# vincentherrmann/constrastive-predictive-coding-audio

Measured on NVIDIA B200. Metric: train audio-sec/sec, higher is better.
Workload: dtype f32

## Files before the change

### constrastive-predictive-coding-audio_b200/cpc_b200/ops.py

```python
import contextlib
import ctypes

import torch
from torch.autograd.function import once_differentiable

from . import _lib

_PRECISION = {"fp32": 0, "bf16": 1}
_default_precision = "fp32"


def set_default_precision(name):
    global _default_precision
    if name not in _PRECISION:
        raise ValueError(name)
    _default_precision = name


def get_default_precision():
    return _default_precision


def strict_fp32_libraries():
    torch.backends.cudnn.allow_tf32 = False
    torch.backends.cuda.matmul.allow_tf32 = False


_second_order = False


@contextlib.contextmanager
def second_order(enabled=True):
    global _second_order
    previous, _second_order = _second_order, bool(enabled)
    try:
        yield
    finally:
        _second_order = previous


def second_order_enabled():
    return _second_order


kernel_switches = {}
_CONV_SWITCHES = (("CPC_FORCE_CUDA_CORE_CONV", _lib.CONV_FLAG_CUDA_CORE), ("CPC_NO_TALL_CONV", _lib.CONV_FLAG_NO_TALL),
                  ("CPC_NO_SMALLK_CONV", _lib.CONV_FLAG_NO_SMALLK), ("CPC_NO_FUSED_DGRAD", _lib.CONV_FLAG_NO_FUSED_DGRAD),
                  ("CPC_NO_MMA_SMALL_WGRAD", _lib.CONV_FLAG_NO_MMA_SMALL_WGRAD))


def _switch(name):
    import os
    if name in kernel_switches:
        return bool(kernel_switches[name])
    return os.environ.get(name) == "1"


switch = _switch


def _conv_flags():
    flags = 0
    for name, bit in _CONV_SWITCHES:
        if _switch(name):
            flags |= bit
    return flags


def _require_cuda(*tensors):
    for t in tensors:
        if t is not None and not t.is_cuda:
            raise _lib.CpcError("cpc_b200 ops need CUDA tensors on a B200 (sm_100a); got a %s tensor and there is "
                                "no CPU fallback" % t.device.type)


def _ptr(t):
    return ctypes.c_void_p(t.data_ptr()) if t is not None else ctypes.c_void_p(0)


def _stream():
    return ctypes.c_void_p(torch.cuda.current_stream().cuda_stream)


class KernelProfiler:

    def __init__(self):
        self.records = []

    def __enter__(self):
        global _profiler
        _profiler = self
        return self

    def __exit__(self, *exc):
        global _profiler
        _profiler = None

    def summary(self):
        torch.cuda.synchronize()
        agg = {}
        for key, flops, nbytes, e0, e1 in self.records:
            a = agg.setdefault(key, {"key": key, "count": 0, "total_ms": 0.0, "flops_per_launch": flops,
                                     "bytes_per_launch": nbytes})
            a["count"] += 1
            a["total_ms"] += e0.elapsed_time(e1)
        total = sum(a["total_ms"] for a in agg.values()) or 1.0
        out = sorted(agg.values(), key=lambda a: -a["total_ms"])
        for a in out:
            a["avg_ms"] = a["total_ms"] / a["count"]
            a["share"] = a["total_ms"] / total
            a["tflops"] = a["flops_per_launch"] / (a["avg_ms"] * 1e-3) / 1e12 if a["avg_ms"] > 0 else 0.0
            a["gbs"] = a["bytes_per_launch"] / (a["avg_ms"] * 1e-3) / 1e9 if a["avg_ms"] > 0 else 0.0
        return out


_profiler = None


def _call(key, flops, fn, *args, nbytes=0.0):
    if _profiler is None:
        status = fn(*args)
    else:
        e0, e1 = torch.cuda.Event(enable_timing=True), torch.cuda.Event(enable_timing=True)
        e0.record()
        status = fn(*args)
        e1.record()
        _profiler.records.append((key, flops, nbytes, e0, e1))
    _lib.check(status, key.split(" ")[0])


CONV_FAMILIES = {0: "conv_tiled_cuda_core", 1: "conv_small_k_direct", 2: "tall_conv_tcgen05_32ch", 3: "tall_conv_tcgen05_128ch",
                 4: "conv_implicit_gemm_tcgen05"}


def _conv_key(tag, p):
    which = {"cpc_conv_fwd": 0, "cpc_conv_dgrad": 1, "cpc_conv_wgrad": 2}[tag]
    fam = CONV_FAMILIES.get(_lib.load().cpc_conv_kernel_family(ctypes.byref(p), which), "?")
    return "%s b%d %dx%dx%d->%dx%dx%d k%dx%d s%dx%d [%s]" % (tag, p.batch, p.c_in, p.h_in, p.w_in, p.c_out, p.h_out,
                                                            p.w_out, p.kh, p.kw, p.stride_h, p.stride_w, fam)


def _conv_flops(p):
    return 2.0 * p.c_out * p.c_in * p.kh * p.kw * p.batch * p.h_out * p.w_out


def _workspace(nbytes, device):
    if nbytes == 0:
        return None
    return torch.empty(int(nbytes), dtype=torch.uint8, device=device)



_OVERLAP_MAX_FLOPS = 60e9
_side_streams = {}


def _side_stream(device):
    key = (device.type, device.index)
    if key not in _side_streams:
        _side_streams[key] = torch.cuda.Stream(device=device)
    return _side_streams[key]


def _conv_params(x_shape, w_shape, stride, pad_top, pad_left, out_hw, relu, precision):
    p = _lib.ConvParams()
    p.batch, p.c_in, p.h_in, p.w_in = x_shape
    p.c_out, _, p.kh, p.kw = w_shape
    p.h_out, p.w_out = out_hw
    p.stride_h, p.stride_w = stride
    p.pad_top, p.pad_left = pad_top, pad_left
    p.relu = int(relu)
    p.precision = _PRECISION[precision]
    p.flags = _conv_flags()
    return p


def _pack_operand(lib, t, p, operand):
    nbytes = lib.cpc_conv_packed_bytes(ctypes.byref(p), operand)
    if nbytes == 0:
        return None
    packed = torch.empty(int(nbytes), dtype=torch.uint8, device=t.device)
    _call("cpc_conv_pack %s" % ("x" if operand == 0 else "dy"), 0.0, lib.cpc_conv_pack, _ptr(t), _ptr(packed), ctypes.byref(p),
          operand, _stream(), nbytes=4.0 * t.numel() + float(nbytes))
    return packed


class _ConvFunction(torch.autograd.Function):
    @staticmethod
    def forward(ctx, x, weight, bias, stride, pad_top, pad_left, out_hw, relu, precision):
        y, saved = _conv_forward(ctx, x, weight, bias, stride, pad_top, pad_left, out_hw, relu, precision)
        ctx.save_for_backward(*saved)
        return y

    @staticmethod
    def backward(ctx, dy):
        return _conv_backward(ctx, ctx.saved_tensors, dy) + (None,) * 6


class _ConvPoolFunction(torch.autograd.Function):

    @staticmethod
    def forward(ctx, x, weight, bias, stride, pad_top, pad_left, out_hw, relu, precision, kernel, ceil_mode):
        y, saved = _conv_forward(ctx, x, weight, bias, stride, pad_top, pad_left, out_hw, relu, precision)
        lib = _lib.load()
        x = saved[0]
        p = _pool_params(tuple(x.shape), kernel, ceil_mode)
        if p.h_out <= 0 or p.w_out <= 0:
            raise ValueError("max_pool2d output would be empty for input %s, kernel %d" % (tuple(x.shape), kernel))
        pooled = torch.empty((p.batch, p.channels, p.h_out, p.w_out), dtype=torch.float32, device=x.device)
        with torch.cuda.device(x.device):
            _call("cpc_maxpool_fwd b%d %dx%dx%d k%d" % (p.batch, p.channels, p.h_in, p.w_in, kernel), 0.0,
                  lib.cpc_maxpool_fwd, _ptr(x), _ptr(pooled), ctypes.byref(p), _stream(),
                  nbytes=4.0 * (x.numel() + pooled.numel()))
        ctx.pool = (kernel, ceil_mode)
        ctx.set_materialize_grads(False)
        ctx.save_for_backward(*saved)
        return y, pooled

    @staticmethod
    @once_differentiable
    def backward(ctx, dy, d_pooled):
        saved = ctx.saved_tensors
        x = saved[0]
        kernel, ceil_mode = ctx.pool
        lib = _lib.load()
        dx = dw = db = None
        if dy is not None:
            dx, dw, db = _conv_backward(ctx, saved, dy)
        if d_pooled is not None and ctx.needs_input_grad[0]:
            p = _pool_params(tuple(x.shape), kernel, ceil_mode)
            d_pooled = d_pooled.contiguous()
            with torch.cuda.device(x.device):
                if dx is None:
                    dx = torch.empty_like(x)
                    _call("cpc_maxpool_bwd b%d %dx%dx%d k%d" % (p.batch, p.channels, p.h_in, p.w_in, kernel), 0.0,
                          lib.cpc_maxpool_bwd, _ptr(x), _ptr(d_pooled), _ptr(dx), ctypes.byref(p), _stream(),
                          nbytes=4.0 * (2 * x.numel() + d_pooled.numel()))
                else:
                    _call("cpc_maxpool_bwd b%d %dx%dx%d k%d +=" % (p.batch, p.channels, p.h_in, p.w_in, kernel), 0.0,
                          lib.cpc_maxpool_bwd_accumulate, _ptr(x), _ptr(d_pooled), _ptr(dx), ctypes.byref(p), _stream(),
                          nbytes=4.0 * (3 * x.numel() + d_pooled.numel()))
        return (dx, dw, db) + (None,) * 8


def _conv_forward(ctx, x, weight, bias, stride, pad_top, pad_left, out_hw, relu, precision):
    _require_cuda(x, weight, bias)
    lib = _lib.load()
    x = x.contiguous()
    w = weight.contiguous()
    if x.dtype != torch.float32 or w.dtype != torch.float32:
        raise _lib.CpcError("conv expects fp32 tensors (precision is a kernel-internal setting)")
    p = _conv_params(tuple(x.shape), tuple(w.shape), stride, pad_top, pad_left, out_hw, relu, precision)
    y = torch.empty((x.shape[0], w.shape[0], out_hw[0], out_hw[1]), dtype=torch.float32, device=x.device)
    ws = _workspace(lib.cpc_conv_workspace_bytes(ctypes.byref(p), 0), x.device)
    with torch.cuda.device(x.device):
        keep = ctx.needs_input_grad[1]
        packed_x = _pack_operand(lib, x, p, 0) if keep else None
        _call(_conv_key("cpc_conv_fwd", p), _conv_flops(p), lib.cpc_conv_fwd_ex, _ptr(x), _ptr(w),
              _ptr(bias.contiguous() if bias is not None else None), _ptr(y), ctypes.byref(p), _ptr(packed_x),
              _ptr(ws), ws.numel() if ws is not None else 0, _stream())
    ctx.params = (tuple(x.shape), tuple(w.shape), stride, pad_top, pad_left, out_hw, precision)
    ctx.has_bias = bias is not None
    ctx.relu = relu
    return y, (x, w, y if relu else None, packed_x)


def _conv_backward(ctx, saved, dy):
    x, w, y, packed_x = saved
    lib = _lib.load()
    x_shape, w_shape, stride, pad_top, pad_left, out_hw, precision = ctx.params
    if ctx.relu:
        dy = dy * (y > 0).to(dy.dtype) if torch.is_grad_enabled() else torch.ops.aten.threshold_backward(dy, y, 0.0)
    dy = dy.contiguous()
    if torch.is_grad_enabled():
        geom = (x_shape, w_shape, stride, pad_top, pad_left, out_hw, precision)
        dx = _ConvDgradFunction.apply(dy, w, geom) if ctx.needs_input_grad[0] else None
        dw = _ConvWgradFunction.apply(x, dy, geom) if ctx.needs_input_grad[1] else None
        db = dy.sum(dim=(0, 2, 3)) if (ctx.has_bias and ctx.needs_input_grad[2]) else None
        return dx, dw, db
    p = _conv_params(x_shape, w_shape, stride, pad_top, pad_left, out_hw, False, precision)
    dx = dw = db = None
    need_dx = ctx.needs_input_grad[0]
    need_dw = ctx.needs_input_grad[1] or (ctx.has_bias and ctx.needs_input_grad[2])
    with torch.cuda.device(dy.device):
        packed_dy = None
        if need_dw:
            nbytes = lib.cpc_conv_packed_bytes(ctypes.byref(p), 1)
            if nbytes and ctx.has_bias:
                packed_dy = torch.empty(int(nbytes), dtype=torch.uint8, device=dy.device)
                db = torch.empty(w_shape[0], dtype=torch.float32, device=dy.device)
                _call("cpc_conv_pack dy", 0.0, lib.cpc_conv_pack_dy, _ptr(dy), _ptr(packed_dy), _ptr(db), ctypes.byref(p),
                      _stream(), nbytes=4.0 * dy.numel() + float(nbytes))
            else:
                packed_dy = _pack_operand(lib, dy, p, 1)
        side = None
        if need_dx and need_dw and _profiler is None and _conv_flops(p) < _OVERLAP_MAX_FLOPS and not _switch("CPC_NO_BWD_OVERLAP"):
            side = _side_stream(dy.device)
            side.wait_stream(torch.cuda.current_stream(dy.device))
        ws_d = ws_w = None
        if need_dx:
            dx = torch.empty(x_shape, dtype=torch.float32, device=dy.device)
            ws_d = _workspace(lib.cpc_conv_workspace_bytes(ctypes.byref(p), 1), dy.device)
            _call(_conv_key("cpc_conv_dgrad", p), _conv_flops(p), lib.cpc_conv_dgrad_ex, _ptr(dy), _ptr(w), _ptr(dx),
                  ctypes.byref(p), _ptr(packed_dy), _ptr(ws_d), ws_d.numel() if ws_d is not None else 0, _stream())
        if need_dw:
            dw = torch.empty(w_shape, dtype=torch.float32, device=dy.device)
            db_here = None
            if ctx.has_bias and db is None:
                db = db_here = torch.empty(w_shape[0], dtype=torch.float32, device=dy.device)
            ws_w = _workspace(lib.cpc_conv_workspace_bytes(ctypes.byref(p), 2), dy.device)
            with (torch.cuda.stream(side) if side is not None else contextlib.nullcontext()):
                _call(_conv_key("cpc_conv_wgrad", p), _conv_flops(p), lib.cpc_conv_wgrad_ex, _ptr(x), _ptr(dy), _ptr(dw),
                      _ptr(db_here), ctypes.byref(p), _ptr(packed_x), _ptr(packed_dy), _ptr(ws_w),
                      ws_w.numel() if ws_w is not None else 0, _stream())
        if side is not None:
            torch.cuda.current_stream(dy.device).wait_stream(side)
    return dx, dw, db


class _ConvDgradFunction(torch.autograd.Function):

    @staticmethod
    def forward(ctx, dy, w, geom):
        _require_cuda(dy, w)
        lib = _lib.load()
        x_shape, w_shape, stride, pad_top, pad_left, out_hw, precision = geom
        dy, w = dy.contiguous(), w.contiguous()
        p = _conv_params(x_shape, w_shape, stride, pad_top, pad_left, out_hw, False, precision)
        dx = torch.empty(x_shape, dtype=torch.float32, device=dy.device)
        ws = _workspace(lib.cpc_conv_workspace_bytes(ctypes.byref(p), 1), dy.device)
        with torch.cuda.device(dy.device):
            _call(_conv_key("cpc_conv_dgrad", p), _conv_flops(p), lib.cpc_conv_dgrad_ex, _ptr(dy), _ptr(w), _ptr(dx),
                  ctypes.byref(p), _ptr(None), _ptr(ws), ws.numel() if ws is not None else 0, _stream())
        ctx.geom = geom
        ctx.save_for_backward(dy, w)
        return dx

    @staticmethod
    def backward(ctx, g):
        dy, w = ctx.saved_tensors
        x_shape, w_shape, stride, pad_top, pad_left, out_hw, precision = ctx.geom
        g = g.contiguous()
        g_dy = (_ConvFunction.apply(g, w, None, stride, pad_top, pad_left, out_hw, False, precision)
                if ctx.needs_input_grad[0] else None)
        g_w = _ConvWgradFunction.apply(g, dy, ctx.geom) if ctx.needs_input_grad[1] else None
        return g_dy, g_w, None


class _ConvWgradFunction(torch.autograd.Function):

    @staticmethod
    def forward(ctx, x, dy, geom):
        _require_cuda(x, dy)
        lib = _lib.load()
        x_shape, w_shape, stride, pad_top, pad_left, out_hw, precision = geom
        x, dy = x.contiguous(), dy.contiguous()
        p = _conv_params(x_shape, w_shape, stride, pad_top, pad_left, out_hw, False, precision)
        dw = torch.empty(w_shape, dtype=torch.float32, device=dy.device)
        ws = _workspace(lib.cpc_conv_workspace_bytes(ctypes.byref(p), 2), dy.device)
        with torch.cuda.device(dy.device):
            _call(_conv_key("cpc_conv_wgrad", p), _conv_flops(p), lib.cpc_conv_wgrad_ex, _ptr(x), _ptr(dy), _ptr(dw),
                  _ptr(None), ctypes.byref(p), _ptr(None), _ptr(None), _ptr(ws), ws.numel() if ws is not None else 0,
                  _stream())
        ctx.geom = geom
        ctx.save_for_backward(x, dy)
        return dw

    @staticmethod
    def backward(ctx, g):
        x, dy = ctx.saved_tensors
        x_shape, w_shape, stride, pad_top, pad_left, out_hw, precision = ctx.geom
        g = g.contiguous()
        g_x = _ConvDgradFunction.apply(dy, g, ctx.geom) if ctx.needs_input_grad[0] else None
        g_dy = (_ConvFunction.apply(x, g, None, stride, pad_top, pad_left, out_hw, False, precision)
                if ctx.needs_input_grad[1] else None)
        return g_x, g_dy, None


def conv2d(x, weight, bias=None, stride=(1, 1), padding=(0, 0), extra_top=0, relu=False, precision=None):
    if isinstance(stride, int):
        stride = (stride, stride)
    if isinstance(padding, int):
        padding = (padding, padding)
    b, c, h, w_in = x.shape
    co, ci, kh, kw = weight.shape
    if ci != c:
        raise ValueError("channel mismatch: input has %d channels, weight expects %d" % (c, ci))
    oh = (h + extra_top + 2 * padding[0] - kh) // stride[0] + 1
    ow = (w_in + 2 * padding[1] - kw) // stride[1] + 1
    if oh <= 0 or ow <= 0:
        raise ValueError("conv output would be empty: input %s kernel %s" % (tuple(x.shape), (kh, kw)))
    return _ConvFunction.apply(x, weight, bias, tuple(stride), extra_top + padding[0], padding[1], (oh, ow), relu,
                               precision or _default_precision)


def conv2d_with_pool(x, weight, bias, stride, padding, extra_top, pool_kernel, pool_ceil_mode, precision=None):
    if isinstance(stride, int):
        stride = (stride, stride)
    if isinstance(padding, int):
        padding = (padding, padding)
    b, c, h, w_in = x.shape
    co, ci, kh, kw = weight.shape
    if ci != c:
        raise ValueError("channel mismatch: input has %d channels, weight expects %d" % (c, ci))
    oh = (h + extra_top + 2 * padding[0] - kh) // stride[0] + 1
    ow = (w_in + 2 * padding[1] - kw) // stride[1] + 1
    if oh <= 0 or ow <= 0:
        raise ValueError("conv output would be empty: input %s kernel %s" % (tuple(x.shape), (kh, kw)))
    return _ConvPoolFunction.apply(x, weight, bias, tuple(stride), extra_top + padding[0], padding[1], (oh, ow), False,
                                   precision or _default_precision, int(pool_kernel), bool(pool_ceil_mode))


def conv1d(x, weight, bias=None, stride=1, padding=0, relu=False, precision=None):
    y = conv2d(x.unsqueeze(2), weight.unsqueeze(2), bias, (1, stride), (0, padding), 0, relu, precision)
    return y.squeeze(2)


def conv_transpose1d(x, weight, stride=1, padding=0, precision=None):
    n, c_in, t = x.shape
    if weight.shape[0] != c_in:
        raise ValueError("channel mismatch: input has %d channels, weight expects %d" % (c_in, weight.shape[0]))
    c_out, k = weight.shape[1], weight.shape[2]
    length = (t - 1) * stride - 2 * padding + k
    if length <= 0:
        raise ValueError("conv_transpose1d output would be empty")
    geom = ((n, c_out, 1, length), (c_in, c_out, 1, k), (1, stride), 0, padding, (1, t), precision or _default_precision)
    return _ConvDgradFunction.apply(x.unsqueeze(2), weight.unsqueeze(2), geom).squeeze(2)



class _DepthwiseConvFunction(torch.autograd.Function):
    @staticmethod
    def forward(ctx, x, weight, stride, pad_top, pad_left, out_hw):
        _require_cuda(x, weight)
        lib = _lib.load()
        x, w = x.contiguous(), weight.contiguous()
        if x.dtype != torch.float32 or w.dtype != torch.float32:
            raise _lib.CpcError("depthwise conv expects fp32 tensors")
        c = x.shape[1]
        p = _conv_params(tuple(x.shape), (c, c, w.shape[2], w.shape[3]), stride, pad_top, pad_left, out_hw, False, "fp32")
        y = torch.empty((x.shape[0], c, out_hw[0], out_hw[1]), dtype=torch.float32, device=x.device)
        taps = w.shape[2] * w.shape[3]
        with torch.cuda.device(x.device):
            _call("cpc_dwconv_fwd b%d %dx%dx%d k%dx%d" % (x.shape[0], c, x.shape[2], x.shape[3], w.shape[2], w.shape[3]),
                  2.0 * taps * y.numel(), lib.cpc_dwconv_fwd, _ptr(x), _ptr(w), _ptr(y), ctypes.byref(p), _stream(),
                  nbytes=4.0 * (x.numel() + y.numel()))
        ctx.geom = (tuple(x.shape), tuple(w.shape), stride, pad_top, pad_left, out_hw)
        ctx.save_for_backward(x, w)
        return y

    @staticmethod
    @once_differentiable
    def backward(ctx, dy):
        x, w = ctx.saved_tensors
        lib = _lib.load()
        x_shape, w_shape, stride, pad_top, pad_left, out_hw = ctx.geom
        c = x_shape[1]
        p = _conv_params(x_shape, (c, c, w_shape[2], w_shape[3]), stride, pad_top, pad_left, out_hw, False, "fp32")
        dy = dy.contiguous()
        dx = dw = None
        tag = "b%d %dx%dx%d k%dx%d" % (x_shape[0], c, x_shape[2], x_shape[3], w_shape[2], w_shape[3])
        with torch.cuda.device(dy.device):
            if ctx.needs_input_grad[0]:
                dx = torch.empty(x_shape, dtype=torch.float32, device=dy.device)
                _call("cpc_dwconv_dgrad " + tag, 0.0, lib.cpc_dwconv_dgrad, _ptr(dy), _ptr(w), _ptr(dx), ctypes.byref(p),
                      _stream(), nbytes=4.0 * (dx.numel() + dy.numel()))
            if ctx.needs_input_grad[1]:
                dw = torch.empty(w_shape, dtype=torch.float32, device=dy.device)
                _call("cpc_dwconv_wgrad " + tag, 0.0, lib.cpc_dwconv_wgrad, _ptr(x), _ptr(dy), _ptr(dw), ctypes.byref(p),
                      _stream(), nbytes=4.0 * (x.numel() + dy.numel()))
        return dx, dw, None, None, None, None


def depthwise_conv2d(x, weight, stride=(1, 1), padding=(0, 0), extra_top=0):
    if isinstance(stride, int):
        stride = (stride, stride)
    if isinstance(padding, int):
        padding = (padding, padding)
    b, c, h, w_in = x.shape
    if weight.shape[0] != c or weight.shape[1] != 1:
        raise ValueError("depthwise weight must be (C, 1, kh, kw) with C = %d, got %s" % (c, tuple(weight.shape)))
    kh, kw = weight.shape[2], weight.shape[3]
    oh = (h + extra_top + 2 * padding[0] - kh) // stride[0] + 1
    ow = (w_in + 2 * padding[1] - kw) // stride[1] + 1
    if oh <= 0 or ow <= 0:
        raise ValueError("conv output would be empty: input %s kernel %s" % (tuple(x.shape), (kh, kw)))
    if _second_order:
        import torch.nn.functional as F
        return F.conv2d(F.pad(x, (0, 0, extra_top, 0)) if extra_top else x, weight, None, stride, padding, groups=c)
    return _DepthwiseConvFunction.apply(x, weight, tuple(stride), extra_top + padding[0], padding[1], (oh, ow))



def _bn_params(x_shape, res_shape, res_off, relu, outer_relu, training, eps, momentum, packed_planes=0):
    p = _lib.BnParams()
    p.packed_planes = int(packed_planes)
    p.batch, p.channels, p.height, p.width = x_shape
    if res_shape is not None:
        p.res_height, p.res_width = res_shape[2], res_shape[3]
        p.res_off_h, p.res_off_w = res_off
    p.relu, p.outer_relu, p.training = int(relu), int(outer_relu), int(training)
    p.eps, p.momentum = float(eps), float(momentum)
    return p


def _bn_mask(lib, p, device):
    if _switch("CPC_NO_BN_MASK"):
        return None
    n = int(lib.cpc_bn_mask_bytes(ctypes.byref(p)))
    return torch.empty(n, dtype=torch.uint8, device=device) if n else None


def _bn_key(tag, p):
    return "%s b%d %dx%dx%d%s" % (tag, p.batch, p.channels, p.height, p.width, " +res" if p.res_height else "")


class _BnReluFunction(torch.autograd.Function):
    @staticmethod
    def forward(ctx, x, gamma, beta, running_mean, running_var, residual, res_off, relu, outer_relu, training, eps,
                momentum):
        _require_cuda(x, gamma, beta, running_mean, running_var, residual)
        lib = _lib.load()
        x = x.contiguous()
        if residual is not None:
            residual = residual.contiguous()
            if residual.shape[:2] != x.shape[:2]:
                raise ValueError("residual %s does not match %s" % (tuple(residual.shape), tuple(x.shape)))
        if x.dtype != torch.float32 or x.dim() != 4:
            raise _lib.CpcError("bn_relu expects a 4-d fp32 tensor")
        p = _bn_params(tuple(x.shape), None if residual is None else tuple(residual.shape), res_off, relu, outer_relu,
                       training, eps, momentum)
        c = x.shape[1]
        out = torch.empty_like(x)
        save_mean = torch.empty(c, dtype=torch.float32, device=x.device)
        save_rstd = torch.empty(c, dtype=torch.float32, device=x.device)
        ws = _workspace(lib.cpc_bn_relu_workspace_bytes(ctypes.byref(p)), x.device)
        n = x.numel()
        mask = _bn_mask(lib, p, x.device) if any(ctx.needs_input_grad) else None
        with torch.cuda.device(x.device):
            _call(_bn_key("cpc_bn_relu_fwd", p), 0.0, lib.cpc_bn_relu_fwd_mask, _ptr(x), _ptr(gamma), _ptr(beta),
                  _ptr(running_mean), _ptr(running_var), _ptr(residual), _ptr(out), _ptr(save_mean), _ptr(save_rstd),
                  _ptr(mask), ctypes.byref(p), _ptr(ws), ws.numel(), _stream(),
                  nbytes=4.0 * n * ((3 if training else 2) + (1 if residual is not None else 0)))
        ctx.cfg = (tuple(x.shape), None if residual is None else tuple(residual.shape), res_off, relu, outer_relu,
                   training, eps, momentum)
        ctx.has_residual = residual is not None
        ctx.save_for_backward(x, gamma, beta, save_mean, save_rstd, residual if mask is None else None, mask)
        return out

    @staticmethod
    @once_differentiable
    def backward(ctx, dout):
        x, gamma, beta, save_mean, save_rstd, residual, mask = ctx.saved_tensors
        lib = _lib.load()
        x_shape, res_shape, res_off, relu, outer_relu, training, eps, momentum = ctx.cfg
        p = _bn_params(x_shape, res_shape, res_off, relu, outer_relu, training, eps, momentum)
        dout = dout.contiguous()
        dx = torch.empty_like(x)
        dgamma = torch.empty_like(gamma) if gamma is not None else None
        dbeta = torch.empty_like(beta) if beta is not None else None
        d_res = (torch.empty(res_shape, dtype=torch.float32, device=x.device)
                 if (ctx.has_residual and ctx.needs_input_grad[5]) else None)
        ws = _workspace(lib.cpc_bn_relu_workspace_bytes(ctypes.byref(p)), x.device)
        n = x.numel()
        res_arg = residual if residual is not None else (x if ctx.has_residual else None)
        with torch.cuda.device(x.device):
            _call(_bn_key("cpc_bn_relu_bwd", p), 0.0, lib.cpc_bn_relu_bwd_mask, _ptr(dout), _ptr(x), _ptr(gamma),
                  _ptr(beta), _ptr(save_mean), _ptr(save_rstd), _ptr(res_arg), _ptr(mask), _ptr(dx), _ptr(dgamma),
                  _ptr(dbeta), _ptr(d_res), ctypes.byref(p), _ptr(ws), ws.numel(), _stream(),
                  nbytes=4.0 * n * (5 + (2 if (residual is not None and outer_relu) else 0) + (1 if d_res is not None else 0))
                  + (2.0 * mask.numel() if mask is not None else 0.0))
        return dx, dgamma, dbeta, None, None, d_res, None, None, None, None, None, None


def bn_relu(x, bn, residual=None, res_off=(0, 0), relu=True, outer_relu=False):
    training = bn.training or bn.running_mean is None
    momentum = bn.momentum
    if training and bn.track_running_stats and bn.num_batches_tracked is not None:
        bn.num_batches_tracked.add_(1)
        if momentum is None:
            momentum = 1.0 / float(bn.num_batches_tracked)
    if momentum is None:
        momentum = 0.0
    rm = bn.running_mean if bn.track_running_stats else None
    rv = bn.running_var if bn.track_running_stats else None
    return _BnReluFunction.apply(x, bn.weight, bn.bias, rm, rv, residual, tuple(res_off), bool(relu), bool(outer_relu),
                                 bool(training), bn.eps, momentum)


def _bn_state(bn):
    training = bn.training or bn.running_mean is None
    momentum = bn.momentum
    if training and bn.track_running_stats and bn.num_batches_tracked is not None:
        bn.num_batches_tracked.add_(1)
        if momentum is None:
            momentum = 1.0 / float(bn.num_batches_tracked)
    if momentum is None:
        momentum = 0.0
    rm = bn.running_mean if bn.track_running_stats else None
    rv = bn.running_var if bn.track_running_stats else None
    return bool(training), momentum, rm, rv


class _BlockTailFunction(torch.autograd.Function):

    @staticmethod
    def forward(ctx, y_a, g0, b0, rm0, rv0, w, bias, g1, b1, rm1, rv1, residual, cfg):
        (top, out_hw, res_off, outer_relu, tr0, eps0, mom0, tr1, eps1, mom1, precision) = cfg
        _require_cuda(y_a, w, residual)
        lib = _lib.load()
        y_a = y_a.contiguous()
        w = w.contiguous()
        if residual is not None:
            residual = residual.contiguous()
        dev = y_a.device
        B, C, H, W = y_a.shape
        planes = 1 if precision == "bf16" else 2
        p0 = _bn_params((B, C, H, W), None, (0, 0), True, False, tr0, eps0, mom0, planes)
        packed_h = torch.empty(int(lib.cpc_bn_packed_bytes(ctypes.byref(p0))), dtype=torch.uint8, device=dev)
        mean0 = torch.empty(C, dtype=torch.float32, device=dev)
        rstd0 = torch.empty(C, dtype=torch.float32, device=dev)
        ws = _workspace(lib.cpc_bn_relu_workspace_bytes(ctypes.byref(p0)), dev)
        pc = _conv_params((B, C, H, W), tuple(w.shape), (1, 1), top, 0, out_hw, False, precision)
        co = w.shape[0]
        y_b = torch.empty((B, co, out_hw[0], out_hw[1]), dtype=torch.float32, device=dev)
        p1 = _bn_params(tuple(y_b.shape), None if residual is None else tuple(residual.shape), res_off, True, outer_relu,
                        tr1, eps1, mom1)
        out = torch.empty_like(y_b)
        mean1 = torch.empty(co, dtype=torch.float32, device=dev)
        rstd1 = torch.empty(co, dtype=torch.float32, device=dev)
        with torch.cuda.device(dev):
            _call(_bn_key("cpc_bn_relu_fwd", p0) + " ->packed", 0.0, lib.cpc_bn_relu_fwd_packed, _ptr(y_a), _ptr(g0), _ptr(b0),
                  _ptr(rm0), _ptr(rv0), _ptr(None), _ptr(packed_h), _ptr(mean0), _ptr(rstd0), ctypes.byref(p0), _ptr(ws),
                  ws.numel(), _stream(), nbytes=4.0 * y_a.numel() * (2 if tr0 else 1) + float(packed_h.numel()))
            wsc = _workspace(lib.cpc_conv_workspace_bytes(ctypes.byref(pc), 0), dev)
            _call(_conv_key("cpc_conv_fwd", pc), _conv_flops(pc), lib.cpc_conv_fwd_ex, _ptr(None), _ptr(w),
                  _ptr(bias.contiguous() if bias is not None else None), _ptr(y_b), ctypes.byref(pc), _ptr(packed_h),
                  _ptr(wsc), wsc.numel() if wsc is not None else 0, _stream())
            ws1 = _workspace(lib.cpc_bn_relu_workspace_bytes(ctypes.byref(p1)), dev)
            n1 = y_b.numel()
            mask = _bn_mask(lib, p1, dev) if any(ctx.needs_input_grad) else None
            _call(_bn_key("cpc_bn_relu_fwd", p1), 0.0, lib.cpc_bn_relu_fwd_mask, _ptr(y_b), _ptr(g1), _ptr(b1), _ptr(rm1),
                  _ptr(rv1), _ptr(residual), _ptr(out), _ptr(mean1), _ptr(rstd1), _ptr(mask), ctypes.byref(p1), _ptr(ws1),
                  ws1.numel(), _stream(), nbytes=4.0 * n1 * ((3 if tr1 else 2) + (1 if residual is not None else 0)))
        ctx.cfg = cfg
        ctx.has_bias = bias is not None
        ctx.res_shape = None if residual is None else tuple(residual.shape)
        ctx.save_for_backward(y_a, g0, b0, mean0, rstd0, packed_h, w, y_b, g1, b1, mean1, rstd1,
                              residual if mask is None else None, mask)
        return out

    @staticmethod
    @once_differentiable
    def backward(ctx, dout):
        y_a, g0, b0, mean0, rstd0, packed_h, w, y_b, g1, b1, mean1, rstd1, residual, mask = ctx.saved_tensors
        (top, out_hw, res_off, outer_relu, tr0, eps0, mom0, tr1, eps1, mom1, precision) = ctx.cfg
        lib = _lib.load()
        dev = dout.device
        dout = dout.contiguous()
        B, C, H, W = y_a.shape
        co = w.shape[0]
        planes = 1 if precision == "bf16" else 2
        p1 = _bn_params(tuple(y_b.shape), ctx.res_shape, res_off, True, outer_relu, tr1, eps1, mom1, planes)
        res_arg = residual if residual is not None else (y_b if ctx.res_shape is not None else None)
        pc = _conv_params((B, C, H, W), tuple(w.shape), (1, 1), top, 0, out_hw, False, precision)
        p0 = _bn_params((B, C, H, W), None, (0, 0), True, False, tr0, eps0, mom0)
        packed_dy = torch.empty(int(lib.cpc_bn_packed_bytes(ctypes.byref(p1))), dtype=torch.uint8, device=dev)
        db = torch.empty(co, dtype=torch.float32, device=dev) if ctx.has_bias else None
        dg1 = torch.empty_like(g1) if g1 is not None else None
        dbt1 = torch.empty_like(b1) if b1 is not None else None
        d_res = (torch.empty(ctx.res_shape, dtype=torch.float32, device=dev)
                 if (ctx.res_shape is not None and ctx.needs_input_grad[11]) else None)
        dh = torch.empty((B, C, H, W), dtype=torch.float32, device=dev)
        dw = torch.empty_like(w)
        dy_a = torch.empty_like(y_a)
        dg0 = torch.empty_like(g0) if g0 is not None else None
        dbt0 = torch.empty_like(b0) if b0 is not None else None
        with torch.cuda.device(dev):
            ws1 = _workspace(lib.cpc_bn_relu_workspace_bytes(ctypes.byref(p1)), dev)
            n1 = y_b.numel()
            _call(_bn_key("cpc_bn_relu_bwd", p1) + " ->packed", 0.0, lib.cpc_bn_relu_bwd_packed_mask, _ptr(dout), _ptr(y_b),
                  _ptr(g1), _ptr(b1), _ptr(mean1), _ptr(rstd1), _ptr(res_arg), _ptr(mask), _ptr(packed_dy), _ptr(db),
                  _ptr(dg1), _ptr(dbt1), _ptr(d_res), ctypes.byref(p1), _ptr(ws1), ws1.numel(), _stream(),
                  nbytes=4.0 * n1 * (5 + (2 if (residual is not None and outer_relu) else 0) + (1 if d_res is not None else 0))
                  + (2.0 * mask.numel() if mask is not None else 0.0))
            wsd = _workspace(lib.cpc_conv_workspace_bytes(ctypes.byref(pc), 1), dev)
            _call(_conv_key("cpc_conv_dgrad", pc), _conv_flops(pc), lib.cpc_conv_dgrad_ex, _ptr(None), _ptr(w), _ptr(dh),
                  ctypes.byref(pc), _ptr(packed_dy), _ptr(wsd), wsd.numel() if wsd is not None else 0, _stream())
            wsw = _workspace(lib.cpc_conv_workspace_bytes(ctypes.byref(pc), 2), dev)
            _call(_conv_key("cpc_conv_wgrad", pc), _conv_flops(pc), lib.cpc_conv_wgrad_ex, _ptr(None), _ptr(None), _ptr(dw),
                  _ptr(None), ctypes.byref(pc), _ptr(packed_h), _ptr(packed_dy), _ptr(wsw),
                  wsw.numel() if wsw is not None else 0, _stream())
            ws0 = _workspace(lib.cpc_bn_relu_workspace_bytes(ctypes.byref(p0)), dev)
            _call(_bn_key("cpc_bn_relu_bwd", p0), 0.0, lib.cpc_bn_relu_bwd, _ptr(dh), _ptr(y_a), _ptr(g0), _ptr(b0), _ptr(mean0),
                  _ptr(rstd0), _ptr(None), _ptr(dy_a), _ptr(dg0), _ptr(dbt0), _ptr(None), ctypes.byref(p0), _ptr(ws0),
                  ws0.numel(), _stream(), nbytes=4.0 * y_a.numel() * 5)
        return dy_a, dg0, dbt0, None, None, dw, db, dg1, dbt1, None, None, d_res, None


def block_tail_eligible(y_a, bn0, conv, top, bn1):
    if _switch("CPC_NO_BLOCK_TAIL") or _second_order:
        return False
    if not (y_a.is_cuda and y_a.dtype == torch.float32 and y_a.dim() == 4 and y_a.shape[3] % 2 == 0):
        return False
    w = conv.weight
    if (tuple(conv.stride) != (1, 1) or w.shape[3] != 1 or conv.padding[1] != 0 or conv.groups != 1
            or tuple(conv.dilation) != (1, 1) or w.shape[1] != y_a.shape[1]):
        return False
    for bn in (bn0, bn1):
        if bn.weight is None or bn.bias is None:
            return False
    B, C, H, W = y_a.shape
    oh = H + top + 2 * conv.padding[0] - w.shape[2] + 1
    if oh <= 0:
        return False
    p = _conv_params((B, C, H, W), tuple(w.shape), (1, 1), top + conv.padding[0], 0, (oh, W), False, _default_precision)
    lib = _lib.load()
    return all(lib.cpc_conv_kernel_family(ctypes.byref(p), which) in (2, 3) for which in (0, 1, 2))


def block_tail(y_a, bn0, conv, top, bn1, residual=None, res_off=(0, 0), outer_relu=False):
    tr0, mom0, rm0, rv0 = _bn_state(bn0)
    tr1, mom1, rm1, rv1 = _bn_state(bn1)
    w = conv.weight
    pad_top = top + conv.padding[0]
    oh = y_a.shape[2] + top + 2 * conv.padding[0] - w.shape[2] + 1
    cfg = (pad_top, (oh, y_a.shape[3]), tuple(res_off), bool(outer_relu), tr0, bn0.eps, mom0, tr1, bn1.eps, mom1,
           _default_precision)
    return _BlockTailFunction.apply(y_a, bn0.weight, bn0.bias, rm0, rv0, w, conv.bias, bn1.weight, bn1.bias, rm1, rv1,
                                    residual, cfg)



def _pool_params(x_shape, kernel, ceil_mode):
    p = _lib.PoolParams()
    p.batch, p.channels, p.h_in, p.w_in = x_shape
    p.kernel, p.ceil_mode = int(kernel), int(bool(ceil_mode))
    p.h_out = -(-p.h_in // kernel) if ceil_mode else p.h_in // kernel
    p.w_out = -(-p.w_in // kernel) if ceil_mode else p.w_in // kernel
    return p


class _MaxPoolFunction(torch.autograd.Function):
    @staticmethod
    def forward(ctx, x, kernel, ceil_mode):
        _require_cuda(x)
        lib = _lib.load()
        x = x.contiguous()
        if x.dtype != torch.float32 or x.dim() != 4:
            raise _lib.CpcError("max_pool2d expects a 4-d fp32 tensor")
        p = _pool_params(tuple(x.shape), kernel, ceil_mode)
        if p.h_out <= 0 or p.w_out <= 0:
            raise ValueError("max_pool2d output would be empty for input %s, kernel %d" % (tuple(x.shape), kernel))
        y = torch.empty((p.batch, p.channels, p.h_out, p.w_out), dtype=torch.float32, device=x.device)
        with torch.cuda.device(x.device):
            _call("cpc_maxpool_fwd b%d %dx%dx%d k%d" % (p.batch, p.channels, p.h_in, p.w_in, kernel), 0.0,
                  lib.cpc_maxpool_fwd, _ptr(x), _ptr(y), ctypes.byref(p), _stream(), nbytes=4.0 * (x.numel() + y.numel()))
        ctx.cfg = (tuple(x.shape), kernel, ceil_mode)
        ctx.save_for_backward(x)
        return y

    @staticmethod
    @once_differentiable
    def backward(ctx, dy):
        (x,) = ctx.saved_tensors
        lib = _lib.load()
        x_shape, kernel, ceil_mode = ctx.cfg
        p = _pool_params(x_shape, kernel, ceil_mode)
        dy = dy.contiguous()
        dx = torch.empty_like(x)
        with torch.cuda.device(x.device):
            _call("cpc_maxpool_bwd b%d %dx%dx%d k%d" % (p.batch, p.channels, p.h_in, p.w_in, kernel), 0.0,
                  lib.cpc_maxpool_bwd, _ptr(x), _ptr(dy), _ptr(dx), ctypes.byref(p), _stream(),
                  nbytes=4.0 * (2 * x.numel() + dy.numel()))
        return dx, None, None


def max_pool2d(x, kernel, ceil_mode=False):
    return _MaxPoolFunction.apply(x, int(kernel), bool(ceil_mode))



def _nce_key(tag, p):
    return "%s b%d k%d e%d %s" % (tag, p.batch, p.steps, p.enc, "all-steps" if p.all_steps else "per-step")


def _nce_pairs_e(p):
    n = p.batch * p.steps
    return float(n * n * p.enc) if p.all_steps else float(p.steps * p.batch * p.batch * p.enc)


def _nce_flops(p):
    return (3.0 if p.score_kind == _lib.SCORE_DIFFERENCE else 2.0) * _nce_pairs_e(p)


def _nce_bwd_flops(p):
    return _nce_flops(p) + 4.0 * _nce_pairs_e(p)


def _nce_params(pred, targets, all_steps, kind, reg, precision):
    p = _lib.InfoNceParams()
    p.batch, p.steps, p.enc = pred.shape
    p.all_steps = int(bool(all_steps))
    p.score_kind = {"linear": _lib.SCORE_LINEAR, "softplus": _lib.SCORE_SOFTPLUS,
                    "difference": _lib.SCORE_DIFFERENCE}[kind]
    p.regularization = float(reg)
    p.tgt_stride_b, p.tgt_stride_e, p.tgt_stride_k = targets.stride()
    p.precision = _PRECISION[precision]
    p.flags = _lib.INFONCE_FLAG_NO_TENSOR if _switch("CPC_NO_TENSOR_INFONCE") else 0
    return p


class _InfoNceFunction(torch.autograd.Function):
    @staticmethod
    def forward(ctx, pred, targets, all_steps, kind, reg, precision):
        _require_cuda(pred, targets)
        lib = _lib.load()
        if pred.dtype != torch.float32 or targets.dtype != torch.float32:
            raise _lib.CpcError("infonce expects fp32 tensors")
        b, k, e = pred.shape
        if tuple(targets.shape) != (b, e, k):
            raise ValueError("targets must be (B, E, K) = %s, got %s" % ((b, e, k), tuple(targets.shape)))
        pred = pred.contiguous()
        p = _nce_params(pred, targets, all_steps, kind, reg, precision)
        out = torch.empty(_lib.INFONCE_OUT_FLOATS, dtype=torch.float32, device=pred.device)
        lse = torch.empty(b * k, dtype=torch.float32, device=pred.device)
        ws = _workspace(lib.cpc_infonce_workspace_bytes(ctypes.byref(p), 0), pred.device)
        with torch.cuda.device(pred.device):
            _call(_nce_key("cpc_infonce_fwd", p), _nce_flops(p), lib.cpc_infonce_fwd, _ptr(pred), _ptr(targets),
                  _ptr(out), _ptr(lse), ctypes.byref(p), _ptr(ws), ws.numel() if ws is not None else 0, _stream())
        ctx.args = (all_steps, kind, reg, precision)
        ctx.save_for_backward(pred, targets, lse)
        loss, max_score, loss_noreg, mean_score = out[0], out[1], out[2], out[3]
        ctx.mark_non_differentiable(max_score, loss_noreg, mean_score)
        return loss, max_score, loss_noreg, mean_score

    @staticmethod
    @once_differentiable
    def backward(ctx, g_loss, _g1, _g2, _g3):
        pred, targets, lse = ctx.saved_tensors
        lib = _lib.load()
        all_steps, kind, reg, precision = ctx.args
        p = _nce_params(pred, targets, all_steps, kind, reg, precision)
        g = g_loss.reshape(1).to(torch.float32).contiguous()
        d_pred = torch.empty_like(pred)
        d_tgt = torch.empty(targets.shape, dtype=torch.float32, device=pred.device)
        ws = _workspace(lib.cpc_infonce_workspace_bytes(ctypes.byref(p), 1), pred.device)
        with torch.cuda.device(pred.device):
            _call(_nce_key("cpc_infonce_bwd", p), _nce_bwd_flops(p), lib.cpc_infonce_bwd, _ptr(pred), _ptr(targets),
                  _ptr(lse), _ptr(g), _ptr(d_pred), _ptr(d_tgt), ctypes.byref(p), _ptr(ws),
                  ws.numel() if ws is not None else 0, _stream())
        return d_pred, d_tgt, None, None, None, None


def infonce(pred, targets, all_steps, kind="linear", regularization=0.0, precision=None):
    return _InfoNceFunction.apply(pred, targets, bool(all_steps), kind, float(regularization),
                                  precision or _default_precision)


def infonce_validate(pred, targets, all_steps, kind="linear", precision=None):
    _require_cuda(pred, targets)
    lib = _lib.load()
    if pred.dtype != torch.float32 or targets.dtype != torch.float32:
        raise _lib.CpcError("infonce_validate expects fp32 tensors")
    b, k, e = pred.shape
    if tuple(targets.shape) != (b, e, k):
        raise ValueError("targets must be (B, E, K) = %s, got %s" % ((b, e, k), tuple(targets.shape)))
    pred = pred.detach().contiguous()
    targets = targets.detach()
    p = _nce_params(pred, targets, all_steps, kind, 0.0, precision or _default_precision)
    metrics = torch.empty(2 * k + 1, dtype=torch.float32, device=pred.device)
    ws = _workspace(lib.cpc_infonce_workspace_bytes(ctypes.byref(p), 2), pred.device)
    with torch.cuda.device(pred.device):
        _call(_nce_key("cpc_infonce_validate", p), _nce_flops(p), lib.cpc_infonce_validate, _ptr(pred), _ptr(targets),
              _ptr(metrics), ctypes.byref(p), _ptr(ws), ws.numel(), _stream())
    return metrics[:k], metrics[k:2 * k], metrics[2 * k]



def _cqt_params(plan, batch, n_samples, x_pitch, n_frames, mode, pool_t, eps, log_offset, norm, power):
    p = _lib.CqtParams()
    p.batch, p.n_samples, p.x_pitch = batch, n_samples, x_pitch
    p.n_bins, p.hop, p.n_frames = plan["n_bins"], plan["hop"], n_frames
    p.n_groups = len(plan["kernel_sizes"])
    for g, (ks, (lo, hi), wo) in enumerate(zip(plan["kernel_sizes"], plan["ranges"], plan["weight_offsets"])):
        p.kernel_size[g], p.bin_lo[g], p.bin_hi[g], p.weight_offset[g] = ks, lo, hi, wo
    p.mode, p.pool_t = mode, pool_t
    p.eps, p.log_offset, p.norm, p.power = eps, log_offset, norm, power
    p.flags = _lib.CQT_FLAG_NO_TENSOR if _switch("CPC_NO_TENSOR_CQT") else 0
    if _default_precision == "bf16":
        p.flags |= _lib.CQT_FLAG_HALF_OPERANDS
    import os
    p.flags |= (int(kernel_switches.get("CPC_CQT_ROUND", os.environ.get("CPC_CQT_ROUND", "0"))) & 0xff) << 8
    return p


def cqt_pack_filters(weights, plan):
    _require_cuda(weights)
    lib = _lib.load()
    k0 = plan["kernel_sizes"][0]
    p = _cqt_params(plan, 1, k0 + 1, k0 + 1, 1, _lib.CQT_COMPLEX, 1, 0.0, 0.0, 1.0, 1.0)
    p.flags = 0
    nbytes = lib.cpc_cqt_packed_filter_bytes(ctypes.byref(p))
    if nbytes == 0:
        return None
    packed = torch.empty(int(nbytes), dtype=torch.uint8, device=weights.device)
    with torch.cuda.device(weights.device):
        _call("cpc_cqt_pack_filters", 0.0, lib.cpc_cqt_pack_filters, _ptr(weights), _ptr(packed), ctypes.byref(p), _stream())
    return packed


def cqt_frontend(x, weights, plan, mode, phase_fixed=None, phase_scale=None, pool_t=1, eps=0.0, log_offset=0.0,
                 norm=1.0, power=1.0, packed_filters=None):
    _require_cuda(x, weights)
    lib = _lib.load()
    if x.dim() == 3:
        if x.shape[1] != 1:
            raise ValueError("CQT expects mono input (B,1,L)")
        x = x[:, 0]
    x = x.contiguous()
    if x.dtype != torch.float32:
        raise _lib.CpcError("CQT expects fp32 audio")
    b, l = x.shape
    k0 = plan["kernel_sizes"][0]
    t = (l - 1 - k0) // plan["hop"] + 1
    if t <= 0:
        raise ValueError("input of %d samples is shorter than the CQT receptive field %d (+1)" % (l, k0))
    p = _cqt_params(plan, b, l, x.stride(0), t, mode, pool_t, eps, log_offset, norm, power)
    f = plan["n_bins"]
    if mode == _lib.CQT_COMPLEX:
        out = torch.empty((b, f, t, 2), dtype=torch.float32, device=x.device)
    elif mode == _lib.CQT_LOGPOW:
        out = torch.empty((b, 1, f, t // pool_t), dtype=torch.float32, device=x.device)
    else:
        if t < 2:
            raise ValueError("phase mode needs at least 2 CQT frames")
        out = torch.empty((b, 2, f, (t - 1) // pool_t), dtype=torch.float32, device=x.device)
    ws = _workspace(lib.cpc_cqt_workspace_bytes(ctypes.byref(p)), x.device)
    with torch.cuda.device(x.device):
        taps = sum(2 * (hi - lo) * ks for ks, (lo, hi) in zip(plan["kernel_sizes"], plan["ranges"]))
        c_out = 2 if mode == _lib.CQT_LOGPOW_PHASE else (2 if mode == _lib.CQT_COMPLEX else 1)
        _call("cpc_cqt_fwd b%d L%d T%d mode%d" % (b, l, t, mode), 2.0 * taps * b * t, lib.cpc_cqt_fwd_ex, _ptr(x),
              _ptr(weights), _ptr(packed_filters), _ptr(phase_fixed), _ptr(phase_scale), _ptr(out), ctypes.byref(p), _ptr(ws),
              ws.numel() if ws is not None else 0, _stream(), nbytes=4.0 * b * l + 4.0 * out.numel())
    return out
```

### constrastive-predictive-coding-audio_b200/csrc/conv.cu

```cuda
#include "common.cuh"

#include <cuda_bf16.h>
#include <cstdlib>

namespace cpc {

size_t umma_conv_workspace(const cpc_conv_params* p, int which);
bool umma_conv_eligible(const cpc_conv_params* p, int which);
int umma_conv_launch(const float* in, const float* w, const float* bias, float* out, const cpc_conv_params* p, int which,
                     const void* pre, void* workspace, size_t workspace_bytes, cudaStream_t s);
int pack_split_launch(const float* x, __nv_bfloat16* out, long rows, int W, int Wp, int planes, int nrep, int w_mul,
                      int rep_mul, int w_off, cudaStream_t s);
int pack_split_sum_launch(const float* x, __nv_bfloat16* out, float* sums, long rows, int W, int Wp, int planes, int H, int C,
                          int nrep, cudaStream_t s);
int umma_dy_replicas(const cpc_conv_params* p);

size_t umma_wgrad_workspace(const cpc_conv_params* p);
bool umma_wgrad_eligible(const cpc_conv_params* p);
int umma_wgrad_launch(const float* x, const float* dy, float* dw, const cpc_conv_params* p, const void* pre_x,
                      const void* pre_dy, void* workspace, size_t workspace_bytes, cudaStream_t s);

size_t tall_conv_workspace(const cpc_conv_params* p, int which);
bool tall_conv_eligible(const cpc_conv_params* p, int which);
int tall_conv_launch(const float* in, const float* w, const float* bias, float* out, const cpc_conv_params* p, int which,
                     const void* pre, void* workspace, size_t workspace_bytes, cudaStream_t s);
int tall_wgrad_launch(const float* x, const float* dy, float* dw, const cpc_conv_params* p, const void* pre_x,
                      const void* pre_dy, void* workspace, size_t workspace_bytes, cudaStream_t s);

bool smallk_eligible(const cpc_conv_params* p, int which);
int smallk_launch(int which, const float* x, const float* w, const float* bias, const float* dy, float* out,
                  const cpc_conv_params* p, cudaStream_t s);
bool small_dgrad_eligible(const cpc_conv_params* p);
int small_dgrad_launch(const float* dy, const float* w, float* dx, const cpc_conv_params* p, cudaStream_t s);
static bool smallk_path(const cpc_conv_params* p, int which) {
    if (p->flags & CPC_CONV_FLAG_NO_SMALLK) return false;
    return smallk_eligible(p, which);
}

size_t tall128_workspace(const cpc_conv_params* p, int which);
bool tall128_eligible(const cpc_conv_params* p, int which);
int tall128_conv_launch(const float* in, const float* w, const float* bias, float* out, const cpc_conv_params* p, int which,
                        const void* pre, void* workspace, size_t workspace_bytes, cudaStream_t s);
int tall128_wgrad_launch(const float* x, const float* dy, float* dw, const cpc_conv_params* p, const void* pre_x,
                         const void* pre_dy, void* workspace, size_t workspace_bytes, cudaStream_t s);

static int tall_path(const cpc_conv_params* p, int which) {
    if (p->flags & (CPC_CONV_FLAG_CUDA_CORE | CPC_CONV_FLAG_NO_TALL)) return 0;
    if (tall_conv_eligible(p, which)) return 1;
    if (tall128_eligible(p, which)) return 2;
    return 0;
}

static bool tensor_core_path(const cpc_conv_params* p, int which) {
    if (p->flags & CPC_CONV_FLAG_CUDA_CORE) return false;
    return which == 2 ? umma_wgrad_eligible(p) : umma_conv_eligible(p, which);
}

struct ConvGeom {
    int B, Cin, H, W, Cout, OH, OW, kh, kw, sh, sw, pt, pl;
    int khkw, ohow, hw;
    FastDiv d_ow, d_ohow, d_kw, d_khkw, d_w, d_hw, d_sh, d_sw;
};

static ConvGeom make_geom(const cpc_conv_params* p) {
    ConvGeom g;
    g.B = p->batch; g.Cin = p->c_in; g.H = p->h_in; g.W = p->w_in;
    g.Cout = p->c_out; g.OH = p->h_out; g.OW = p->w_out;
    g.kh = p->kh; g.kw = p->kw; g.sh = p->stride_h; g.sw = p->stride_w;
    g.pt = p->pad_top; g.pl = p->pad_left;
    g.khkw = g.kh * g.kw; g.ohow = g.OH * g.OW; g.hw = g.H * g.W;
    g.d_ow = FastDiv(g.OW); g.d_ohow = FastDiv(g.ohow); g.d_kw = FastDiv(g.kw); g.d_khkw = FastDiv(g.khkw);
    g.d_w = FastDiv(g.W); g.d_hw = FastDiv(g.hw); g.d_sh = FastDiv(g.sh); g.d_sw = FastDiv(g.sw);
    return g;
}

static int validate(const cpc_conv_params* p) {
    if (!p) return CPC_ERR_NULL;
    if (p->batch <= 0 || p->c_in <= 0 || p->h_in <= 0 || p->w_in <= 0 || p->c_out <= 0 || p->h_out <= 0 ||
        p->w_out <= 0 || p->kh <= 0 || p->kw <= 0 || p->stride_h <= 0 || p->stride_w <= 0 || p->pad_top < 0 ||
        p->pad_left < 0)
        return CPC_ERR_BAD_SHAPE;
    const int64_t lim = (1ll << 31) - 1;
    if ((int64_t)p->batch * p->h_out * p->w_out > lim || (int64_t)p->batch * p->h_in * p->w_in > lim ||
        (int64_t)p->c_in * p->kh * p->kw > lim || (int64_t)p->c_out * p->kh * p->kw > lim)
        return CPC_ERR_BAD_SHAPE;
    return CPC_OK;
}

struct FwdA {
    static constexpr bool kFast = false;
    const float* x; ConvGeom g; int M, K;
    __device__ __forceinline__ float load(int m, int k) const {
        if (m >= M || k >= K) return 0.f;
        int b, pix, oh, ow, ci, r, i, j;
        g.d_ohow.divmod(m, b, pix);
        g.d_ow.divmod(pix, oh, ow);
        g.d_khkw.divmod(k, ci, r);
        g.d_kw.divmod(r, i, j);
        const int h = oh * g.sh - g.pt + i, w = ow * g.sw - g.pl + j;
        if ((unsigned)h >= (unsigned)g.H || (unsigned)w >= (unsigned)g.W) return 0.f;
        return __ldg(x + ((size_t)(b * g.Cin + ci) * g.H + h) * g.W + w);
    }
};
struct DenseRows {
    static constexpr bool kFast = true;
    const float* w; int N, K;
    __device__ __forceinline__ float load(int n, int k) const {
        if (n >= N || k >= K) return 0.f;
        return __ldg(w + (size_t)n * K + k);
    }
};
struct DgradA {
    static constexpr bool kFast = false;
    const float* dy; ConvGeom g; int M, K;
    __device__ __forceinline__ float load(int m, int k) const {
        if (m >= M || k >= K) return 0.f;
        int b, pix, ih, iw, co, r, i, j;
        g.d_hw.divmod(m, b, pix);
        g.d_w.divmod(pix, ih, iw);
        g.d_khkw.divmod(k, co, r);
        g.d_kw.divmod(r, i, j);
        const int th = ih + g.pt - i, tw = iw + g.pl - j;
        if (th < 0 || tw < 0) return 0.f;
        const int oh = g.d_sh.div(th), ow = g.d_sw.div(tw);
        if (oh * g.sh != th || ow * g.sw != tw || oh >= g.OH || ow >= g.OW) return 0.f;
        return __ldg(dy + ((size_t)(b * g.Cout + co) * g.OH + oh) * g.OW + ow);
    }
};
struct DgradB {
    static constexpr bool kFast = true;
    const float* w; ConvGeom g; int N, K;
    __device__ __forceinline__ float load(int n, int k) const {
        if (n >= N || k >= K) return 0.f;
        int co, r;
        g.d_khkw.divmod(k, co, r);
        return __ldg(w + ((size_t)co * g.Cin + n) * g.khkw + r);
    }
};
struct WgradA {
    static constexpr bool kFast = true;
    const float* dy; ConvGeom g; int M, K;
    __device__ __forceinline__ float load(int m, int k) const {
        if (m >= M || k >= K) return 0.f;
        int b, pix;
        g.d_ohow.divmod(k, b, pix);
        return __ldg(dy + (size_t)(b * g.Cout + m) * g.ohow + pix);
    }
};
struct WgradB {
    static constexpr bool kFast = true;
    const float* x; ConvGeom g; int N, K;
    __device__ __forceinline__ float load(int n, int k) const {
        if (n >= N || k >= K) return 0.f;
        int b, pix, oh, ow, ci, r, i, j;
        g.d_ohow.divmod(k, b, pix);
        g.d_ow.divmod(pix, oh, ow);
        g.d_khkw.divmod(n, ci, r);
        g.d_kw.divmod(r, i, j);
        const int h = oh * g.sh - g.pt + i, w = ow * g.sw - g.pl + j;
        if ((unsigned)h >= (unsigned)g.H || (unsigned)w >= (unsigned)g.W) return 0.f;
        return __ldg(x + ((size_t)(b * g.Cin + ci) * g.H + h) * g.W + w);
    }
};

__global__ void __launch_bounds__(TILE_THREADS) conv_fwd_kernel(FwdA la, DenseRows lb, const float* __restrict__ bias,
                                                               float* __restrict__ y, int relu) {
    __shared__ TileSmem sm;
    const int row0 = blockIdx.x * TILE, col0 = blockIdx.y * TILE;
    float acc[4][4] = {};
    tile_gemm(la, lb, row0, col0, 0, la.K, acc, sm);
    const int tx = threadIdx.x & 15, ty = threadIdx.x >> 4;
    const ConvGeom& g = la.g;
#pragma unroll
    for (int i = 0; i < 4; ++i) {
        const int m = row0 + tx * 4 + i;
        if (m >= la.M) continue;
        int b, pix;
        g.d_ohow.divmod(m, b, pix);
#pragma unroll
        for (int j = 0; j < 4; ++j) {
            const int n = col0 + ty * 4 + j;
            if (n >= lb.N) continue;
            float v = acc[i][j] + (bias ? __ldg(bias + n) : 0.f);
            if (relu) v = fmaxf(v, 0.f);
            y[(size_t)(b * g.Cout + n) * g.ohow + pix] = v;
        }
    }
}

__global__ void __launch_bounds__(TILE_THREADS) conv_dgrad_kernel(DgradA la, DgradB lb, float* __restrict__ dx) {
    __shared__ TileSmem sm;
    const int row0 = blockIdx.x * TILE, col0 = blockIdx.y * TILE;
    float acc[4][4] = {};
    tile_gemm(la, lb, row0, col0, 0, la.K, acc, sm);
    const int tx = threadIdx.x & 15, ty = threadIdx.x >> 4;
    const ConvGeom& g = la.g;
#pragma unroll
    for (int i = 0; i < 4; ++i) {
        const int m = row0 + tx * 4 + i;
        if (m >= la.M) continue;
        int b, pix;
        g.d_hw.divmod(m, b, pix);
#pragma unroll
        for (int j = 0; j < 4; ++j) {
            const int n = col0 + ty * 4 + j;
            if (n >= lb.N) continue;
            dx[(size_t)(b * g.Cin + n) * g.hw + pix] = acc[i][j];
        }
    }
}

__global__ void __launch_bounds__(TILE_THREADS) conv_wgrad_kernel(WgradA la, WgradB lb, float* __restrict__ dw,
                                                                 int k_per_split) {
    __shared__ TileSmem sm;
    const int row0 = blockIdx.x * TILE, col0 = blockIdx.y * TILE;
    const int k_begin = blockIdx.z * k_per_split;
    const int k_end = min(la.K, k_begin + k_per_split);
    float acc[4][4] = {};
    tile_gemm(la, lb, row0, col0, k_begin, k_end, acc, sm);
    const int tx = threadIdx.x & 15, ty = threadIdx.x >> 4;
#pragma unroll
    for (int i = 0; i < 4; ++i) {
        const int m = row0 + tx * 4 + i;
        if (m >= la.M) continue;
#pragma unroll
        for (int j = 0; j < 4; ++j) {
            const int n = col0 + ty * 4 + j;
            if (n >= lb.N) continue;
            atomicAdd(dw + (size_t)m * lb.N + n, acc[i][j]);
        }
    }
}

constexpr int DB_THREADS = 256;
constexpr int DB_PER_THREAD = 16;
__global__ void __launch_bounds__(DB_THREADS) conv_dbias_kernel(const float* __restrict__ dy, float* __restrict__ dbias,
                                                               int Cout, int ohow) {
    const int plane = blockIdx.x;
    const float* p = dy + (size_t)plane * ohow;
    const int i0 = blockIdx.y * (DB_THREADS * DB_PER_THREAD) + threadIdx.x;
    float s = 0.f;
#pragma unroll
    for (int u = 0; u < DB_PER_THREAD; ++u) {
        const int i = i0 + u * DB_THREADS;
        if (i < ohow) s += __ldg(p + i);
    }
    __shared__ float red[8];
    s = warp_sum(s);
    if ((threadIdx.x & 31) == 0) red[threadIdx.x >> 5] = s;
    __syncthreads();
    if (threadIdx.x < 32) {
        float v = threadIdx.x < 8 ? red[threadIdx.x] : 0.f;
        v = warp_sum(v);
        if (threadIdx.x == 0) atomicAdd(dbias + plane % Cout, v);
    }
}

}

using namespace cpc;

extern "C" size_t cpc_conv_workspace_bytes(const cpc_conv_params* p, int which) {
    if (validate(p) != CPC_OK) return 0;
    if ((which == 0 || which == 2) && smallk_path(p, which)) return 0;
    if (which >= 0 && which <= 2 && tall_path(p, which))
        return tall_path(p, which) == 1 ? tall_conv_workspace(p, which) : tall128_workspace(p, which);
    if ((which == 0 || which == 1) && tensor_core_path(p, which)) return umma_conv_workspace(p, which);
    if (which == 2 && tensor_core_path(p, 2)) return umma_wgrad_workspace(p);
    return 0;
}

static int conv_family(const cpc_conv_params* p, int which) {
    if ((which == 0 || which == 2) && smallk_path(p, which)) return 1;
    if (which == 1 && !(p->flags & CPC_CONV_FLAG_NO_SMALLK) && small_dgrad_eligible(p)) return 1;
    if (const int tp = tall_path(p, which)) return tp == 1 ? 2 : 3;
    return tensor_core_path(p, which) ? 4 : 0;
}

extern "C" int cpc_conv_kernel_family(const cpc_conv_params* p, int which) {
    if (validate(p) != CPC_OK || which < 0 || which > 2) return -1;
    return conv_family(p, which);
}

static int dy_replicas(const cpc_conv_params* p) { return conv_family(p, 1) == 4 ? umma_dy_replicas(p) : 1; }

extern "C" size_t cpc_conv_packed_bytes(const cpc_conv_params* p, int operand) {
    if (validate(p) != CPC_OK) return 0;
    const size_t planes = p->precision == 1 ? 1 : 2;
    const size_t Wp = (size_t)((p->w_out + 7) & ~7);
    if (operand == 0) {
        if (conv_family(p, 0) < 2 && conv_family(p, 2) < 2) return 0;
        return align_up(planes * p->kw * p->batch * p->c_in * p->h_in * Wp * 2, 1024);
    }
    if (operand == 1) {
        if (conv_family(p, 2) < 2) return 0;
        const size_t nrep = dy_replicas(p);
        const size_t Wd = (size_t)((p->w_out + (nrep == 2 ? 1 : 0) + 7) & ~7);
        return align_up(planes * nrep * p->batch * p->c_out * p->h_out * Wd * 2, 1024);
    }
    return 0;
}

extern "C" int cpc_conv_pack(const float* src, void* packed, const cpc_conv_params* p, int operand, void* stream) {
    int st = validate(p);
    if (st != CPC_OK) return st;
    if (!src || !packed) return CPC_ERR_NULL;
    if (cpc_conv_packed_bytes(p, operand) == 0) return CPC_ERR_UNSUPPORTED;
    if ((reinterpret_cast<uintptr_t>(packed) & 15) != 0) return CPC_ERR_ALIGNMENT;
    if ((st = check_device()) != CPC_OK) return st;
    const int planes = p->precision == 1 ? 1 : 2;
    const int Wp = (p->w_out + 7) & ~7;
    __nv_bfloat16* out = reinterpret_cast<__nv_bfloat16*>(packed);
    if (operand == 0)
        st = pack_split_launch(src, out, (long)p->batch * p->c_in * p->h_in, p->w_in, Wp, planes, p->kw, p->stride_w, 1,
                               -p->pad_left, (cudaStream_t)stream);
    else {
        const int nrep = dy_replicas(p);
        const int Wd = (p->w_out + (nrep == 2 ? 1 : 0) + 7) & ~7;
        st = pack_split_launch(src, out, (long)p->batch * p->c_out * p->h_out, p->w_out, Wd, planes, nrep, 1, -1, 0,
                               (cudaStream_t)stream);
    }
    if (st == CPC_OK) count_launch();
    return st;
}

extern "C" int cpc_conv_pack_dy(const float* dy, void* packed, float* dbias, const cpc_conv_params* p, void* stream) {
    if (!dbias) return cpc_conv_pack(dy, packed, p, 1, stream);
    int st = validate(p);
    if (st != CPC_OK) return st;
    if (!dy || !packed) return CPC_ERR_NULL;
    if (cpc_conv_packed_bytes(p, 1) == 0) return CPC_ERR_UNSUPPORTED;
    if ((reinterpret_cast<uintptr_t>(packed) & 15) != 0) return CPC_ERR_ALIGNMENT;
    if ((st = check_device()) != CPC_OK) return st;
    const int planes = p->precision == 1 ? 1 : 2;
    const int nrep = dy_replicas(p);
    const int Wp = (p->w_out + (nrep == 2 ? 1 : 0) + 7) & ~7;
    st = pack_split_sum_launch(dy, reinterpret_cast<__nv_bfloat16*>(packed), dbias, (long)p->batch * p->c_out * p->h_out,
                               p->w_out, Wp, planes, p->h_out, p->c_out, nrep, (cudaStream_t)stream);
    if (st == CPC_OK) count_launch();
    return st;
}

extern "C" int cpc_conv_fwd(const float* x, const float* w, const float* bias, float* y, const cpc_conv_params* p,
                            void* workspace, size_t workspace_bytes, void* stream) {
    return cpc_conv_fwd_ex(x, w, bias, y, p, nullptr, workspace, workspace_bytes, stream);
}
extern "C" int cpc_conv_dgrad(const float* dy, const float* w, float* dx, const cpc_conv_params* p, void* workspace,
                              size_t workspace_bytes, void* stream) {
    return cpc_conv_dgrad_ex(dy, w, dx, p, nullptr, workspace, workspace_bytes, stream);
}
extern "C" int cpc_conv_wgrad(const float* x, const float* dy, float* dw, float* dbias, const cpc_conv_params* p,
                              void* workspace, size_t workspace_bytes, void* stream) {
    return cpc_conv_wgrad_ex(x, dy, dw, dbias, p, nullptr, nullptr, workspace, workspace_bytes, stream);
}

extern "C" int cpc_conv_fwd_ex(const float* x, const float* w, const float* bias, float* y, const cpc_conv_params* p,
                               const void* packed_x, void* workspace, size_t workspace_bytes, void* stream) {
    int st = validate(p);
    if (st != CPC_OK) return st;
    {
        const int fam = conv_family(p, 0);
        const bool packed_only = !x && packed_x && (fam == 2 || fam == 3);
        if ((!x && !packed_only) || !w || !y) return CPC_ERR_NULL;
    }
    if ((st = check_device()) != CPC_OK) return st;
    cudaStream_t s = (cudaStream_t)stream;
    switch (conv_family(p, 0)) {
        case 1: return smallk_launch(0, x, w, bias, nullptr, y, p, s);
        case 2: return tall_conv_launch(x, w, bias, y, p, 0, packed_x, workspace, workspace_bytes, s);
        case 3: return tall128_conv_launch(x, w, bias, y, p, 0, packed_x, workspace, workspace_bytes, s);
        case 4: return umma_conv_launch(x, w, bias, y, p, 0, packed_x, workspace, workspace_bytes, s);
        default: break;
    }
    ConvGeom g = make_geom(p);
    const int M = g.B * g.ohow, N = g.Cout, K = g.Cin * g.khkw;
    FwdA la{x, g, M, K};
    DenseRows lb{w, N, K};
    dim3 grid(ceil_div(M, TILE), ceil_div(N, TILE));
    conv_fwd_kernel<<<grid, TILE_THREADS, 0, s>>>(la, lb, bias, y, p->relu);
    CPC_LAUNCH_CHECK();
    count_launch();
    return CPC_OK;
}

extern "C" int cpc_conv_dgrad_ex(const float* dy, const float* w, float* dx, const cpc_conv_params* p, const void* packed_dy,
                                 void* workspace, size_t workspace_bytes, void* stream) {
    int st = validate(p);
    if (st != CPC_OK) return st;
    {
        const int fam = conv_family(p, 1);
        const bool packed_only = !dy && packed_dy && (fam == 2 || fam == 3);
        if ((!dy && !packed_only) || !w || !dx) return CPC_ERR_NULL;
    }
    if ((st = check_device()) != CPC_OK) return st;
    cudaStream_t s = (cudaStream_t)stream;
    switch (conv_family(p, 1)) {
        case 1: return small_dgrad_launch(dy, w, dx, p, s);
        case 2: return tall_conv_launch(dy, w, nullptr, dx, p, 1, packed_dy, workspace, workspace_bytes, s);
        case 3: return tall128_conv_launch(dy, w, nullptr, dx, p, 1, packed_dy, workspace, workspace_bytes, s);
        case 4: return umma_conv_launch(dy, w, nullptr, dx, p, 1, packed_dy, workspace, workspace_bytes, s);
        default: break;
    }
    ConvGeom g = make_geom(p);
    const int M = g.B * g.hw, N = g.Cin, K = g.Cout * g.khkw;
    DgradA la{dy, g, M, K};
    DgradB lb{w, g, N, K};
    dim3 grid(ceil_div(M, TILE), ceil_div(N, TILE));
    conv_dgrad_kernel<<<grid, TILE_THREADS, 0, s>>>(la, lb, dx);
    CPC_LAUNCH_CHECK();
    count_launch();
    return CPC_OK;
}

static int launch_dbias(const float* dy, float* dbias, const ConvGeom& g, cudaStream_t s) {
    if (cudaMemsetAsync(dbias, 0, sizeof(float) * (size_t)g.Cout, s) != cudaSuccess) return CPC_ERR_CUDA;
    const dim3 grid(g.B * g.Cout, ceil_div(g.ohow, DB_THREADS * DB_PER_THREAD));
    conv_dbias_kernel<<<grid, DB_THREADS, 0, s>>>(dy, dbias, g.Cout, g.ohow);
    CPC_LAUNCH_CHECK();
    count_launch();
    return CPC_OK;
}

extern "C" int cpc_conv_wgrad_ex(const float* x, const float* dy, float* dw, float* dbias, const cpc_conv_params* p,
                                 const void* packed_x, const void* packed_dy, void* workspace, size_t workspace_bytes,
                                 void* stream) {
    int st = validate(p);
    if (st != CPC_OK) return st;
    const int fam = conv_family(p, 2);
    {
        const bool tall = fam == 2 || fam == 3;
        if ((!x && !(packed_x && tall)) || (!dy && !(packed_dy && tall && !dbias)) || !dw) return CPC_ERR_NULL;
    }
    if ((st = check_device()) != CPC_OK) return st;
    ConvGeom g = make_geom(p);
    cudaStream_t s = (cudaStream_t)stream;
    if (fam != 0) {
        if (fam == 1) st = smallk_launch(2, x, nullptr, nullptr, dy, dw, p, s);
        else if (fam == 2) st = tall_wgrad_launch(x, dy, dw, p, packed_x, packed_dy, workspace, workspace_bytes, s);
        else if (fam == 3) st = tall128_wgrad_launch(x, dy, dw, p, packed_x, packed_dy, workspace, workspace_bytes, s);
        else st = umma_wgrad_launch(x, dy, dw, p, packed_x, packed_dy, workspace, workspace_bytes, s);
        if (st != CPC_OK) return st;
        return dbias ? launch_dbias(dy, dbias, g, s) : CPC_OK;
    }
    const int M = g.Cout, N = g.Cin * g.khkw, K = g.B * g.ohow;
    if (cudaMemsetAsync(dw, 0, sizeof(float) * (size_t)M * N, s) != cudaSuccess) return CPC_ERR_CUDA;
    const int tiles = ceil_div(M, TILE) * ceil_div(N, TILE);
    int splits = ceil_div(148 * 4, tiles);
    const int max_splits = ceil_div(K, TILE_K * 8);
    if (splits > max_splits) splits = max_splits;
    if (splits < 1) splits = 1;
    int k_per_split = ceil_div(ceil_div(K, splits), TILE_K) * TILE_K;
    splits = ceil_div(K, k_per_split);
    WgradA la{dy, g, M, K};
    WgradB lb{x, g, N, K};
    dim3 grid(ceil_div(M, TILE), ceil_div(N, TILE), splits);
    conv_wgrad_kernel<<<grid, TILE_THREADS, 0, s>>>(la, lb, dw, k_per_split);
    CPC_LAUNCH_CHECK();
    count_launch();
    if (dbias) return launch_dbias(dy, dbias, g, s);
    return CPC_OK;
}
```

### constrastive-predictive-coding-audio_b200/csrc/conv_umma.cu

```cuda
#include <cstdlib>
#include "common.cuh"
#include "umma.cuh"

namespace cpc {
using namespace umma;

constexpr int UM_THREADS = 256;
constexpr int ATOM = 64;
constexpr int KCHUNK = 64;
constexpr int A_PLANE_BYTES = 2 * KCHUNK * 128;
constexpr int SMEM_LIMIT = 227 * 1024;

struct UmmaConv {
    int n_atoms, PH, PW, AW;
    int n_rows_out;
    int n_tile, n_ntiles;
    int th, tw, ntaps, tpc, cin_eff, cin_chunks, n_chunks;
    int h_mul, tap_h_mul, h_off;
    int out_H, out_W, oh_mul, oh_off, ow_mul, ow_off;
    int planes;
    int nrep;
    int srcH;
    int w_resident;
    int fuse;
    int relu, stages;
    const float* bias;
    float* y;
};

__global__ void __launch_bounds__(256) pack_split_kernel(const float* __restrict__ x, __nv_bfloat16* __restrict__ out,
                                                        long rows, int W, int Wp, int planes, int nrep, int w_mul,
                                                        int rep_mul, int w_off, int vec_ok) {
    const int groups = Wp >> 3;
    const long total = rows * groups;
    const long plane_stride = (long)nrep * rows * Wp;
    for (long g = (long)blockIdx.x * blockDim.x + threadIdx.x; g < total; g += (long)gridDim.x * blockDim.x) {
        const long row = g / groups;
        const int w0 = (int)(g - row * groups) << 3;
        const float* src = x + row * W;
        if (w_mul == 2 && rep_mul == 1 && nrep == 3) {
            const int wb = 2 * w0 + w_off;
            if (wb >= 0 && wb + 17 <= W) {
                float win[17];
                if (vec_ok && !(wb & 1)) {
#pragma unroll
                    for (int i = 0; i < 8; ++i) {
                        const float2 t = __ldg(reinterpret_cast<const float2*>(src + wb) + i);
                        win[2 * i] = t.x; win[2 * i + 1] = t.y;
                    }
                    win[16] = __ldg(src + wb + 16);
                } else {
#pragma unroll
                    for (int i = 0; i < 17; ++i) win[i] = __ldg(src + wb + i);
                }
                __nv_bfloat16 whi[17], wlo[17];
#pragma unroll
                for (int i = 0; i < 17; ++i) {
                    whi[i] = __float2bfloat16_rn(win[i]);
                    wlo[i] = __float2bfloat16_rn(win[i] - __bfloat162float(whi[i]));
                }
#pragma unroll
                for (int r = 0; r < 3; ++r) {
                    __align__(16) __nv_bfloat16 hi[8];
                    __align__(16) __nv_bfloat16 lo[8];
#pragma unroll
                    for (int i = 0; i < 8; ++i) { hi[i] = whi[2 * i + r]; lo[i] = wlo[2 * i + r]; }
                    const long o = ((long)r * rows + row) * Wp + w0;
                    *reinterpret_cast<uint4*>(out + o) = *reinterpret_cast<const uint4*>(hi);
                    if (planes == 2) *reinterpret_cast<uint4*>(out + plane_stride + o) = *reinterpret_cast<const uint4*>(lo);
                }
                continue;
            }
        }
        for (int r = 0; r < nrep; ++r) {
            __align__(16) __nv_bfloat16 hi[8];
            __align__(16) __nv_bfloat16 lo[8];
            const int wb = w_mul * w0 + rep_mul * r + w_off;
            float v[8];
            if (vec_ok && w_mul == 1 && !(wb & 1) && wb >= 0 && wb + 8 <= W) {
#pragma unroll
                for (int i = 0; i < 4; ++i) {
                    const float2 t = __ldg(reinterpret_cast<const float2*>(src + wb) + i);
                    v[2 * i] = t.x; v[2 * i + 1] = t.y;
                }
            } else {
#pragma unroll
                for (int i = 0; i < 8; ++i) {
                    const int w = wb + w_mul * i;
                    v[i] = (w >= 0 && w < W) ? __ldg(src + w) : 0.f;
                }
            }
#pragma unroll
            for (int i = 0; i < 8; ++i) {
                hi[i] = __float2bfloat16_rn(v[i]);
                lo[i] = __float2bfloat16_rn(v[i] - __bfloat162float(hi[i]));
            }
            const long o = ((long)r * rows + row) * Wp + w0;
            *reinterpret_cast<uint4*>(out + o) = *reinterpret_cast<const uint4*>(hi);
            if (planes == 2) *reinterpret_cast<uint4*>(out + plane_stride + o) = *reinterpret_cast<const uint4*>(lo);
        }
    }
}

constexpr int PACK_BINS = 264;
__global__ void __launch_bounds__(256) pack_split_sum_kernel(const float* __restrict__ x, __nv_bfloat16* __restrict__ out,
                                                            float* __restrict__ sums, long rows, int W, int Wp, int planes,
                                                            FastDiv d_h, FastDiv d_groups, int C, int vec_ok, int nrep) {
    __shared__ float bins[2][PACK_BINS];
    const int groups = Wp >> 3, lane = threadIdx.x & 31;
    const long total = rows * groups;
    const long rep_stride = rows * (long)Wp;
    const long plane_stride = nrep * rep_stride;
    for (int t = threadIdx.x; t < 2 * PACK_BINS; t += 256) (&bins[0][0])[t] = 0.f;
    __syncthreads();
    const long n_iter = (total + (long)gridDim.x * 256 - 1) / ((long)gridDim.x * 256);
    for (long it = 0; it < n_iter; ++it) {
        float* bin = bins[it & 1];
        const long g0 = (it * gridDim.x + blockIdx.x) * 256;
        const long g = g0 + threadIdx.x;
        const int plane_first = d_h.div(d_groups.div((int)min(g0, total - 1)));
        int plane = -1;
        float sum = 0.f;
        if (g < total) {
            int row, gi;
            d_groups.divmod((int)g, row, gi);
            const int w0 = gi << 3;
            plane = d_h.div(row);
            const float* src = x + (long)row * W;
            float v[8];
            if (vec_ok && w0 + 8 <= W) {
#pragma unroll
                for (int i = 0; i < 4; ++i) {
                    const float2 t = __ldg(reinterpret_cast<const float2*>(src + w0) + i);
                    v[2 * i] = t.x; v[2 * i + 1] = t.y;
                }
            } else {
#pragma unroll
                for (int i = 0; i < 8; ++i) v[i] = (w0 + i < W) ? __ldg(src + w0 + i) : 0.f;
            }
            __align__(16) __nv_bfloat16 hi[8];
            __align__(16) __nv_bfloat16 lo[8];
#pragma unroll
            for (int i = 0; i < 8; ++i) {
                sum += v[i];
                hi[i] = __float2bfloat16_rn(v[i]);
                lo[i] = __float2bfloat16_rn(v[i] - __bfloat162float(hi[i]));
            }
            const long o = (long)row * Wp + w0;
            *reinterpret_cast<uint4*>(out + o) = *reinterpret_cast<const uint4*>(hi);
            if (planes == 2) *reinterpret_cast<uint4*>(out + plane_stride + o) = *reinterpret_cast<const uint4*>(lo);
            if (nrep == 2) {
                const float vp = (w0 > 0 && w0 - 1 < W) ? __ldg(src + w0 - 1) : 0.f;
                __align__(16) __nv_bfloat16 h1[8];
                __align__(16) __nv_bfloat16 l1[8];
                h1[0] = __float2bfloat16_rn(vp);
                l1[0] = __float2bfloat16_rn(vp - __bfloat162float(h1[0]));
#pragma unroll
                for (int i = 1; i < 8; ++i) { h1[i] = hi[i - 1]; l1[i] = lo[i - 1]; }
                *reinterpret_cast<uint4*>(out + rep_stride + o) = *reinterpret_cast<const uint4*>(h1);
                if (planes == 2) *reinterpret_cast<uint4*>(out + plane_stride + rep_stride + o) = *reinterpret_cast<const uint4*>(l1);
            }
        }
#pragma unroll
        for (int o = 1; o < 32; o <<= 1) {
            const float t = __shfl_up_sync(0xffffffffu, sum, o);
            const int q = __shfl_up_sync(0xffffffffu, plane, o);
            if (lane >= o && q == plane) sum += t;
        }
        const int next = __shfl_down_sync(0xffffffffu, plane, 1);
        if (plane >= 0 && (lane == 31 || next != plane)) atomicAdd(&bin[plane - plane_first], sum);
        __syncthreads();
        if (g0 < total) {
            const int plane_last = d_h.div(d_groups.div((int)min(g0 + 255, total - 1)));
            for (int t = threadIdx.x; t <= plane_last - plane_first; t += 256) {
                atomicAdd(sums + (plane_first + t) % C, bin[t]);
                bin[t] = 0.f;
            }
        }
    }
}

int pack_split_sum_launch(const float* x, __nv_bfloat16* out, float* sums, long rows, int W, int Wp, int planes, int H, int C,
                          int nrep, cudaStream_t s) {
    if (cudaMemsetAsync(sums, 0, sizeof(float) * (size_t)C, s) != cudaSuccess) return CPC_ERR_CUDA;
    const long groups = rows * (Wp / 8);
    int blocks = (int)((groups + 255) / 256);
    if (blocks > 148 * 16) blocks = 148 * 16;
    if (blocks < 1) blocks = 1;
    const int vec_ok = (W % 2 == 0) && (reinterpret_cast<uintptr_t>(x) % 8 == 0);
    if (groups >= (1l << 31)) return CPC_ERR_BAD_SHAPE;
    pack_split_sum_kernel<<<blocks, 256, 0, s>>>(x, out, sums, rows, W, Wp, planes, FastDiv(H), FastDiv(Wp / 8), C, vec_ok, nrep);
    return cudaGetLastError() == cudaSuccess ? CPC_OK : CPC_ERR_CUDA;
}

int pack_split_launch(const float* x, __nv_bfloat16* out, long rows, int W, int Wp, int planes, int nrep, int w_mul,
                      int rep_mul, int w_off, cudaStream_t s) {
    const long groups = rows * (Wp / 8);
    int blocks = (int)((groups + 255) / 256);
    if (blocks > 148 * 16) blocks = 148 * 16;
    if (blocks < 1) blocks = 1;
    const int vec_ok = (W % 2 == 0) && (reinterpret_cast<uintptr_t>(x) % 8 == 0);
    pack_split_kernel<<<blocks, 256, 0, s>>>(x, out, rows, W, Wp, planes, nrep, w_mul, rep_mul, w_off, vec_ok);
    return cudaGetLastError() == cudaSuccess ? CPC_OK : CPC_ERR_CUDA;
}

struct TapMap { int th, tw, i_off, i_mul, j_off, j_mul, swap, fuse; };

__global__ void __launch_bounds__(256) pack_weights_kernel(const float* __restrict__ w, __nv_bfloat16* __restrict__ out,
                                                          int Cin, int kh, int kw, int n_rows, int k_ch, int cin_eff,
                                                          int cin_chunks, int tpc, int n_chunks, int planes, TapMap tm) {
    const long total = (long)n_chunks * n_rows * KCHUNK;
    const int ntaps = tm.th * tm.tw;
    for (long idx = (long)blockIdx.x * blockDim.x + threadIdx.x; idx < total; idx += (long)gridDim.x * blockDim.x) {
        const int kk = (int)(idx % KCHUNK);
        const long t = idx / KCHUNK;
        const int n = (int)(t % n_rows);
        const int chunk = (int)(t / n_rows);
        int tap, c;
        if (cin_eff == KCHUNK) { tap = chunk / cin_chunks; c = (chunk - tap * cin_chunks) * KCHUNK + kk; }
        else                   { tap = chunk * tpc + kk / cin_eff; c = kk % cin_eff; }
        float v = 0.f;
        if (tap < ntaps && c < k_ch) {
            const int ti = tap / tm.tw, tj = tap - ti * tm.tw;
            if (tm.fuse) {
                const int cls = n / tm.fuse, ci = n - cls * tm.fuse;
                const int i = (cls >> 1) + 2 * ti, j = (cls & 1) + 2 * tj;
                if (i < kh && j < kw) v = __ldg(w + (((size_t)c * Cin + ci) * kh + i) * kw + j);
            } else {
                const int i = tm.i_off + tm.i_mul * ti, j = tm.j_off + tm.j_mul * tj;
                const size_t co = tm.swap ? c : n, ci = tm.swap ? n : c;
                v = __ldg(w + ((co * Cin + ci) * kh + i) * kw + j);
            }
        }
        const __nv_bfloat16 hi = __float2bfloat16_rn(v);
        out[idx] = hi;
        if (planes == 2) out[total + idx] = __float2bfloat16_rn(v - __bfloat162float(hi));
    }
}

__device__ __forceinline__ void umma_live_chunks(const UmmaConv& p, int row0, int row1, int& q_begin, int& q_end) {
    int i_lo = p.th, i_hi = -1;
    const int rows[2] = {row0, row1};
#pragma unroll
    for (int a = 0; a < 2; ++a) {
        const int r = rows[a];
        int lo, hi;
        if (p.tap_h_mul > 0) { lo = max(0, -r); hi = min(p.th - 1, p.srcH - 1 - r); }
        else                 { lo = max(0, r - (p.srcH - 1)); hi = min(p.th - 1, r); }
        if (lo <= hi) { i_lo = min(i_lo, lo); i_hi = max(i_hi, hi); }
    }
    if (i_hi < i_lo) { q_begin = 0; q_end = 1; return; }
    const int t_lo = i_lo * p.tw, t_hi = (i_hi + 1) * p.tw;
    if (p.cin_eff == KCHUNK) { q_begin = t_lo * p.cin_chunks; q_end = t_hi * p.cin_chunks; }
    else { q_begin = t_lo / p.tpc; q_end = (t_hi + p.tpc - 1) / p.tpc; }
}

struct __align__(8) UmmaBarriers {
    uint64_t full[8], empty[8], acc_full[2], acc_empty[2], wfull;
    uint32_t tmem_base;
};

__global__ void __launch_bounds__(UM_THREADS, 1) umma_conv_kernel(const __grid_constant__ CUtensorMap tmap_a,
                                                                 const __grid_constant__ CUtensorMap tmap_b,
                                                                 const UmmaConv p) {
    extern __shared__ __align__(1024) uint8_t smem_raw[];
    uint8_t* smem = reinterpret_cast<uint8_t*>((reinterpret_cast<uintptr_t>(smem_raw) + 1023) & ~(uintptr_t)1023);
    const int b_plane_bytes = p.n_tile * 128;
    const int w_chunk_bytes = p.planes * b_plane_bytes;
    const int w_res_bytes = p.w_resident ? p.n_chunks * w_chunk_bytes : 0;
    const int stage_bytes = p.planes * A_PLANE_BYTES + (p.w_resident ? 0 : w_chunk_bytes);
    uint8_t* w_res = smem;
    uint8_t* stages_base = smem + w_res_bytes;
    UmmaBarriers* bars = reinterpret_cast<UmmaBarriers*>(stages_base + (size_t)p.stages * stage_bytes);
    const int warp = threadIdx.x >> 5, lane = threadIdx.x & 31;
    const int n_mtiles = (p.n_atoms + 1) >> 1;
    const int n_tiles = n_mtiles * p.n_ntiles;

    if (warp == 0 && lane == 0) {
        prefetch_tmap(&tmap_a);
        prefetch_tmap(&tmap_b);
        for (int s = 0; s < p.stages; ++s) { mbar_init(&bars->full[s], 1); mbar_init(&bars->empty[s], 1); }
        for (int b = 0; b < 2; ++b) { mbar_init(&bars->acc_full[b], 1); mbar_init(&bars->acc_empty[b], 4); }
        mbar_init(&bars->wfull, 1);
        fence_barrier_init();
    }
    if (warp == 2) { tmem_alloc(&bars->tmem_base, 512); tmem_relinquish(); }
    tc_fence_before();
    __syncthreads();
    tc_fence_after();
    const uint32_t tmem_base = bars->tmem_base;

    if (warp == 0) {
        if (p.w_resident) {
            if (lane == 0) mbar_expect_tx(&bars->wfull, (uint32_t)w_res_bytes);
            __syncwarp();
            for (int l = lane; l < p.n_chunks * p.planes; l += 32) {
                const int q = l / p.planes, pl = l - q * p.planes;
                tma_load_4d(w_res + q * w_chunk_bytes + pl * b_plane_bytes, &tmap_b, &bars->wfull, 0, 0, q, pl);
            }
        }
        const int taps_per_load = p.cin_eff == KCHUNK ? 1 : p.tpc;
        const int n_a_loads = p.planes * 2 * taps_per_load;
        const int n_loads = n_a_loads + (p.w_resident ? 0 : p.planes);
        const bool is_a = lane < n_a_loads, is_b = !is_a && lane < n_loads;
        const int my_t = is_a ? lane % taps_per_load : 0;
        const int my_a = is_a ? (lane / taps_per_load) & 1 : 0;
        const int my_pl = is_a ? lane / (2 * taps_per_load) : lane - n_a_loads;
        const uint32_t my_off = is_a ? (uint32_t)(my_pl * A_PLANE_BYTES + my_a * (KCHUNK * 128) + my_t * p.cin_eff * 128)
                                     : (uint32_t)(p.planes * A_PLANE_BYTES + my_pl * b_plane_bytes);
        const int my_rep = my_pl * p.nrep;
        int stage = 0; uint32_t phase = 0;
        for (int tile = blockIdx.x; tile < n_tiles; tile += gridDim.x) {
            const int mtile = tile / p.n_ntiles, ntile = tile - mtile * p.n_ntiles;
            int aoh[2], my_b = 0, my_w0 = 0, my_row = 0;
            for (int a = 0; a < 2; ++a) {
                const int atom = mtile * 2 + a;
                const int row = atom / p.AW;
                const int b = row / p.PH;
                aoh[a] = (row - b * p.PH) * p.h_mul + p.h_off;
                if (a == my_a) { my_b = b; my_w0 = (atom - row * p.AW) * ATOM; my_row = aoh[a]; }
            }
            int q_begin, q_end;
            umma_live_chunks(p, aoh[0], aoh[1], q_begin, q_end);
            int ti, tj, cc = 0;
            {
                const int tap0 = p.cin_eff == KCHUNK ? q_begin / p.cin_chunks : q_begin * p.tpc + my_t;
                if (p.cin_eff == KCHUNK) cc = q_begin - tap0 * p.cin_chunks;
                ti = tap0 / p.tw; tj = tap0 - ti * p.tw;
            }
            for (int q = q_begin; q < q_end; ++q) {
                if (lane == 0) {
                    mbar_wait(&bars->empty[stage], phase ^ 1);
                    mbar_expect_tx(&bars->full[stage], (uint32_t)stage_bytes);
                }
                __syncwarp();
                uint8_t* dst = stages_base + (size_t)stage * stage_bytes + my_off;
                if (is_a) {
                    const bool phantom = ti >= p.th;
                    tma_load_5d(dst, &tmap_a, &bars->full[stage], my_w0, my_row + (phantom ? 0 : ti * p.tap_h_mul),
                                cc * KCHUNK, my_b, my_rep + (phantom ? 0 : tj));
                } else if (is_b) {
                    tma_load_4d(dst, &tmap_b, &bars->full[stage], 0, ntile * p.n_tile, q, my_pl);
                }
                if (p.cin_eff == KCHUNK) {
                    if (++cc == p.cin_chunks) { cc = 0; if (++tj == p.tw) { tj = 0; ++ti; } }
                } else {
                    tj += p.tpc;
                    while (tj >= p.tw) { tj -= p.tw; ++ti; }
                }
                if (++stage == p.stages) { stage = 0; phase ^= 1; }
            }
        }
    } else if (warp == 1) {
        {
            const uint32_t idesc = make_idesc_bf16(128, p.n_tile,  1,  0);
            int stage = 0; uint32_t phase = 0;
            int buf = 0; uint32_t acc_phase = 0;
            if (p.w_resident) { mbar_wait(&bars->wfull, 0); tc_fence_after(); }
            for (int tile = blockIdx.x; tile < n_tiles; tile += gridDim.x) {
                mbar_wait(&bars->acc_empty[buf], acc_phase ^ 1);
                tc_fence_after();
                const uint32_t d_tmem = tmem_base + (uint32_t)buf * 256;
                int aoh[2];
                {
                    const int mtile = tile / p.n_ntiles;
                    for (int a = 0; a < 2; ++a) {
                        const int row = (mtile * 2 + a) / p.AW;
                        aoh[a] = (row - (row / p.PH) * p.PH) * p.h_mul + p.h_off;
                    }
                }
                int q_begin, q_end;
                umma_live_chunks(p, aoh[0], aoh[1], q_begin, q_end);
                for (int q = q_begin; q < q_end; ++q) {
                    mbar_wait(&bars->full[stage], phase);
                    tc_fence_after();
                    const uint32_t st = smem_u32(stages_base + (size_t)stage * stage_bytes);
                    const uint32_t b0 = p.w_resident ? smem_u32(w_res + q * w_chunk_bytes) : st + p.planes * A_PLANE_BYTES;
                    const int ncombo = p.planes == 2 ? 3 : 1;
                    if (elect_one()) {
                        for (int cb = 0; cb < ncombo; ++cb) {
                            const uint32_t a_addr = st + (cb == 2 ? A_PLANE_BYTES : 0);
                            const uint32_t b_addr = b0 + (cb == 1 ? b_plane_bytes : 0);
                            const uint64_t ad0 = make_smem_desc(a_addr, KCHUNK * 128, 1024);
                            const uint64_t bd0 = make_smem_desc(b_addr, 16, 1024);
#pragma unroll
                            for (int k = 0; k < KCHUNK / 16; ++k)
                                mma_bf16(d_tmem, ad0 + (uint64_t)(k * ((16 * 128) >> 4)), bd0 + (uint64_t)(k * (32 >> 4)), idesc,
                                         ((q - q_begin) | cb | k) != 0);
                        }
                        tc_commit(&bars->empty[stage]);
                    }
                    __syncwarp();
                    if (++stage == p.stages) { stage = 0; phase ^= 1; }
                }
                if (elect_one()) tc_commit(&bars->acc_full[buf]);
                __syncwarp();
                if (++buf == 2) { buf = 0; acc_phase ^= 1; }
            }
        }
    } else if (warp >= 4) {
        const int ew = warp & 3;
        const int r = ew * 32 + lane;
        int buf = 0; uint32_t acc_phase = 0;
        for (int tile = blockIdx.x; tile < n_tiles; tile += gridDim.x) {
            const int mtile = tile / p.n_ntiles, ntile = tile - mtile * p.n_ntiles;
            const int atom = mtile * 2 + (r >> 6);
            const int row = atom / p.AW;
            const int pw = (atom - row * p.AW) * ATOM + (r & 63);
            const int b = row / p.PH;
            const int oh = (row - b * p.PH) * p.oh_mul + p.oh_off, ow = pw * p.ow_mul + p.ow_off;
            const bool valid = atom < p.n_atoms && pw < p.PW && oh < p.out_H && ow < p.out_W;
            mbar_wait(&bars->acc_full[buf], acc_phase);
            tc_fence_after();
            const uint32_t taddr = tmem_base + ((uint32_t)(ew * 32) << 16) + (uint32_t)buf * 256;
            const size_t chan_stride = (size_t)p.out_H * p.out_W;
            if (p.fuse) {
                const int a = row - b * p.PH;
                const bool in_dom = atom < p.n_atoms && pw < p.PW;
                float* yb = p.y + (size_t)b * p.fuse * chan_stride;
#pragma unroll 1
                for (int rh = 0; rh < 2; ++rh) {
                    uint32_t v0[32], v1[32];
                    tmem_ld32(taddr + (2 * rh) * 32, v0);
                    tmem_ld32(taddr + (2 * rh + 1) * 32, v1);
                    tmem_ld_wait();
                    const int h = 2 * a + rh, w0 = 2 * pw;
                    if (in_dom && h < p.out_H) {
                        float* yo = yb + (size_t)h * p.out_W + w0;
                        const bool ok0 = w0 < p.out_W, ok1 = w0 + 1 < p.out_W;
#pragma unroll
                        for (int c = 0; c < 32; ++c) {
                            if (ok0) yo[(size_t)c * chan_stride] = __uint_as_float(v0[c]);
                            if (ok1) yo[(size_t)c * chan_stride + 1] = __uint_as_float(v1[c]);
                        }
                    }
                }
                tc_fence_before();
                __syncwarp();
                if (lane == 0) mbar_arrive(&bars->acc_empty[buf]);
                if (++buf == 2) { buf = 0; acc_phase ^= 1; }
                continue;
            }
            float* ybase = p.y + ((size_t)b * p.n_rows_out * p.out_H + oh) * p.out_W + ow;
            for (int c0 = 0; c0 < p.n_tile; c0 += 32) {
                uint32_t v[32];
                tmem_ld32(taddr + c0, v);
                tmem_ld_wait();
                if (valid) {
#pragma unroll
                    for (int c = 0; c < 32; ++c) {
                        const int n = ntile * p.n_tile + c0 + c;
                        float f = __uint_as_float(v[c]);
                        if (p.bias) f += __ldg(p.bias + n);
                        if (p.relu) f = fmaxf(f, 0.f);
                        ybase[(size_t)n * chan_stride] = f;
                    }
                }
            }
            tc_fence_before();
            __syncwarp();
            if (lane == 0) mbar_arrive(&bars->acc_empty[buf]);
            if (++buf == 2) { buf = 0; acc_phase ^= 1; }
        }
    }
    tc_fence_before();
    __syncthreads();
    if (warp == 2) { tc_fence_after(); tmem_dealloc(tmem_base, 512); }
}

struct ConvProblem {
    const float* src; int in_ch, srcH, srcW;
    int out_ch;
    TapMap tm;
    int PH, PW;
    int h_mul, tap_h_mul, h_off;
    int w_mul, rep_mul, w_off;
    int out_H, out_W, oh_mul, oh_off, ow_mul, ow_off;
    const __nv_bfloat16* pre; int pre_Wp, pre_nrep;
    int fuse;
};

struct UmmaPlan {
    bool ok;
    int Wp, cin_eff, cin_chunks, tpc, n_chunks, n_tile, n_ntiles, planes, stages, w_resident;
    size_t act_bytes, w_bytes, smem_bytes;
};

static UmmaPlan plan_problem(const ConvProblem& c, int batch, int precision) {
    UmmaPlan u{};
    u.ok = false;
    const int ci = c.in_ch, co = c.out_ch;
    if (!(ci == 16 || ci == 32 || ci % 64 == 0)) return u;
    if (co % 32 != 0 || !(co <= 128 || co % 128 == 0)) return u;
    if (c.PH <= 0 || c.PW <= 0 || c.tm.th <= 0 || c.tm.tw <= 0) return u;
    if ((long)batch * c.PH * ((c.PW + ATOM - 1) / ATOM) > (1l << 30)) return u;
    u.cin_eff = ci >= KCHUNK ? KCHUNK : ci;
    u.cin_chunks = ci >= KCHUNK ? ci / KCHUNK : 1;
    u.tpc = KCHUNK / u.cin_eff;
    const int ntaps = c.tm.th * c.tm.tw;
    u.n_chunks = ci >= KCHUNK ? ntaps * u.cin_chunks : (ntaps + u.tpc - 1) / u.tpc;
    u.n_tile = co <= 128 ? co : 128;
    u.n_ntiles = co / u.n_tile;
    u.planes = precision == 1 ? 1 : 2;
    u.Wp = c.pre ? c.pre_Wp : (c.PW + 7) & ~7;
    int stage_bytes = u.planes * (A_PLANE_BYTES + u.n_tile * 128);
    const long w_all = (long)u.n_chunks * u.planes * u.n_tile * 128;
    u.w_resident = u.n_ntiles == 1 && w_all + 3L * u.planes * A_PLANE_BYTES <= SMEM_LIMIT - 2048;
    long avail = SMEM_LIMIT - 2048;
    if (u.w_resident) { stage_bytes = u.planes * A_PLANE_BYTES; avail -= w_all; }
    u.stages = (int)(avail / stage_bytes);
    if (u.stages > 8) u.stages = 8;
    if (u.stages < 2) return u;
    u.smem_bytes = (size_t)(u.w_resident ? w_all : 0) + (size_t)u.stages * stage_bytes + sizeof(UmmaBarriers) + 1024;
    u.act_bytes = c.pre ? 0 : align_up((size_t)u.planes * c.tm.tw * batch * ci * c.srcH * u.Wp * 2, 1024);
    u.w_bytes = align_up((size_t)u.planes * u.n_chunks * co * KCHUNK * 2, 1024);
    u.ok = true;
    return u;
}

static int run_problem(const ConvProblem& c, const float* w, const float* bias, float* out, const cpc_conv_params* p,
                       int relu, void* workspace, size_t workspace_bytes, cudaStream_t s) {
    const int B = p->batch;
    UmmaPlan u = plan_problem(c, B, p->precision);
    if (!u.ok) return CPC_ERR_UNSUPPORTED;
    if (!workspace || workspace_bytes < u.act_bytes + u.w_bytes + 1024) return CPC_ERR_WORKSPACE;
    uint8_t* ws = reinterpret_cast<uint8_t*>((reinterpret_cast<uintptr_t>(workspace) + 1023) & ~(uintptr_t)1023);
    const __nv_bfloat16* act = c.pre ? c.pre : reinterpret_cast<__nv_bfloat16*>(ws);
    __nv_bfloat16* wp = reinterpret_cast<__nv_bfloat16*>(ws + u.act_bytes);
    const long rows = (long)B * c.in_ch * c.srcH;
    const int nrep = c.pre ? c.pre_nrep : c.tm.tw;
    {
        if (!c.pre && pack_split_launch(c.src, reinterpret_cast<__nv_bfloat16*>(ws), rows, c.srcW, u.Wp, u.planes, c.tm.tw,
                                        c.w_mul, c.rep_mul, c.w_off, s) != CPC_OK)
            return CPC_ERR_CUDA;
        const long wtotal = (long)u.n_chunks * c.out_ch * KCHUNK;
        int wblocks = (int)((wtotal + 255) / 256);
        if (wblocks > 148 * 8) wblocks = 148 * 8;
        pack_weights_kernel<<<wblocks, 256, 0, s>>>(w, wp, p->c_in, p->kh, p->kw, c.out_ch, c.in_ch, u.cin_eff,
                                                    u.cin_chunks, u.tpc, u.n_chunks, u.planes, c.tm);
        CPC_LAUNCH_CHECK();
    }
    CUtensorMap ta, tb;
    {
        const uint64_t dims[5] = {(uint64_t)u.Wp, (uint64_t)c.srcH, (uint64_t)c.in_ch, (uint64_t)B,
                                  (uint64_t)u.planes * nrep};
        const uint64_t row_b = (uint64_t)u.Wp * 2;
        const uint64_t strides[4] = {row_b, row_b * c.srcH, row_b * c.srcH * c.in_ch, row_b * c.srcH * c.in_ch * B};
        const uint32_t box[5] = {ATOM, 1, (uint32_t)u.cin_eff, 1, 1};
        if (!make_tmap_bf16(&ta, act, 5, dims, strides, box)) return CPC_ERR_CUDA;
        const uint64_t wd[4] = {KCHUNK, (uint64_t)c.out_ch, (uint64_t)u.n_chunks, (uint64_t)u.planes};
        const uint64_t wsr[3] = {KCHUNK * 2, (uint64_t)KCHUNK * 2 * c.out_ch, (uint64_t)KCHUNK * 2 * c.out_ch * u.n_chunks};
        const uint32_t wbox[4] = {KCHUNK, (uint32_t)u.n_tile, 1, 1};
        if (!make_tmap_bf16(&tb, wp, 4, wd, wsr, wbox)) return CPC_ERR_CUDA;
    }
    UmmaConv k{};
    k.AW = (c.PW + ATOM - 1) / ATOM;
    k.PH = c.PH; k.PW = c.PW;
    k.n_atoms = B * c.PH * k.AW;
    k.n_rows_out = c.out_ch; k.n_tile = u.n_tile; k.n_ntiles = u.n_ntiles;
    k.th = c.tm.th; k.tw = c.tm.tw; k.ntaps = c.tm.th * c.tm.tw; k.tpc = u.tpc; k.cin_eff = u.cin_eff;
    k.cin_chunks = u.cin_chunks; k.n_chunks = u.n_chunks;
    k.h_mul = c.h_mul; k.tap_h_mul = c.tap_h_mul; k.h_off = c.h_off;
    k.out_H = c.out_H; k.out_W = c.out_W; k.oh_mul = c.oh_mul; k.oh_off = c.oh_off; k.ow_mul = c.ow_mul; k.ow_off = c.ow_off;
    k.fuse = c.fuse;
    k.planes = u.planes; k.nrep = nrep; k.w_resident = u.w_resident; k.relu = relu; k.stages = u.stages; k.bias = bias; k.y = out; k.srcH = c.srcH;
    if (cudaFuncSetAttribute(umma_conv_kernel, cudaFuncAttributeMaxDynamicSharedMemorySize, SMEM_LIMIT) != cudaSuccess)
        return CPC_ERR_CUDA;
    const int n_tiles = ((k.n_atoms + 1) / 2) * k.n_ntiles;
    const int grid = n_tiles < 148 ? n_tiles : 148;
    umma_conv_kernel<<<grid, UM_THREADS, u.smem_bytes, s>>>(ta, tb, k);
    CPC_LAUNCH_CHECK();
    count_launch(c.pre ? 2 : 3);
    return CPC_OK;
}

static ConvProblem fwd_problem(const float* x, const cpc_conv_params* p) {
    ConvProblem c{};
    c.src = x; c.in_ch = p->c_in; c.srcH = p->h_in; c.srcW = p->w_in; c.out_ch = p->c_out;
    c.tm = TapMap{p->kh, p->kw, 0, 1, 0, 1, 0};
    c.PH = p->h_out; c.PW = p->w_out;
    c.h_mul = p->stride_h; c.tap_h_mul = 1; c.h_off = -p->pad_top;
    c.w_mul = p->stride_w; c.rep_mul = 1; c.w_off = -p->pad_left;
    c.out_H = p->h_out; c.out_W = p->w_out; c.oh_mul = 1; c.oh_off = 0; c.ow_mul = 1; c.ow_off = 0;
    return c;
}

static bool dgrad_problem(const float* dy, const cpc_conv_params* p, int rh, int rw, ConvProblem& c, bool& has_taps) {
    const int sh = p->stride_h, sw = p->stride_w;
    c = ConvProblem{};
    c.src = dy; c.in_ch = p->c_out; c.srcH = p->h_out; c.srcW = p->w_out; c.out_ch = p->c_in;
    const int th = rh < p->kh ? (p->kh - rh + sh - 1) / sh : 0;
    const int tw = rw < p->kw ? (p->kw - rw + sw - 1) / sw : 0;
    has_taps = th > 0 && tw > 0;
    c.tm = TapMap{th, tw, rh, sh, rw, sw, 1};
    const int a_min = p->pad_top > rh ? (p->pad_top - rh + sh - 1) / sh : 0;
    const int e_min = p->pad_left > rw ? (p->pad_left - rw + sw - 1) / sw : 0;
    const int a_top = p->h_in - 1 + p->pad_top - rh, e_top = p->w_in - 1 + p->pad_left - rw;
    if (a_top < 0 || e_top < 0) return false;
    c.PH = a_top / sh - a_min + 1; c.PW = e_top / sw - e_min + 1;
    if (c.PH <= 0 || c.PW <= 0) return false;
    c.h_mul = 1; c.tap_h_mul = -1; c.h_off = a_min;
    c.w_mul = 1; c.rep_mul = -1; c.w_off = e_min;
    c.out_H = p->h_in; c.out_W = p->w_in;
    c.oh_mul = sh; c.oh_off = sh * a_min + rh - p->pad_top;
    c.ow_mul = sw; c.ow_off = sw * e_min + rw - p->pad_left;
    return true;
}

static bool channels_ok(int ci, int co) {
    return (ci == 16 || ci == 32 || ci % 64 == 0) && co % 32 == 0 && (co <= 128 || co % 128 == 0);
}

bool umma_conv_eligible(const cpc_conv_params* p, int which) {
    if (p->stride_h > 8 || p->stride_w > 8) return false;
    if (which == 0) return plan_problem(fwd_problem(nullptr, p), p->batch, p->precision).ok;
    if (!channels_ok(p->c_out, p->c_in)) return false;
    for (int rh = 0; rh < p->stride_h; ++rh)
        for (int rw = 0; rw < p->stride_w; ++rw) {
            ConvProblem c; bool taps;
            if (!dgrad_problem(nullptr, p, rh, rw, c, taps) || !taps) continue;
            if (!plan_problem(c, p->batch, p->precision).ok) return false;
        }
    return true;
}

struct DgradShare {
    bool common;
    int n_classes, max_tw, max_pw, w_off;
    size_t act_bytes;
    size_t max_w_bytes;
    size_t max_single;
};

static DgradShare dgrad_share(const cpc_conv_params* p) {
    DgradShare d{};
    d.common = true;
    bool first = true;
    for (int rh = 0; rh < p->stride_h; ++rh)
        for (int rw = 0; rw < p->stride_w; ++rw) {
            ConvProblem c; bool taps;
            if (!dgrad_problem(nullptr, p, rh, rw, c, taps) || !taps) continue;
            UmmaPlan u = plan_problem(c, p->batch, p->precision);
            ++d.n_classes;
            if (first) { d.w_off = c.w_off; first = false; }
            if (c.w_off != d.w_off || c.w_mul != 1) d.common = false;
            if (c.tm.tw > d.max_tw) d.max_tw = c.tm.tw;
            if (c.PW > d.max_pw) d.max_pw = c.PW;
            if (u.w_bytes > d.max_w_bytes) d.max_w_bytes = u.w_bytes;
            if (u.act_bytes + u.w_bytes > d.max_single) d.max_single = u.act_bytes + u.w_bytes;
        }
    const int planes = p->precision == 1 ? 1 : 2;
    const int Wp = (d.max_pw + 7) & ~7;
    d.act_bytes = align_up((size_t)planes * d.max_tw * p->batch * p->c_out * p->h_out * Wp * 2, 1024);
    return d;
}

static bool fused_dgrad_problem(const float* dy, const cpc_conv_params* p, ConvProblem& c) {
    if (p->flags & CPC_CONV_FLAG_NO_FUSED_DGRAD) return false;
    if (p->stride_h != 2 || p->stride_w != 2 || p->pad_top != 0 || p->pad_left != 0) return false;
    if (p->kh < 2 || p->kh > 4 || p->kw < 2 || p->kw > 4 || p->c_in != 32) return false;
    c = ConvProblem{};
    c.src = dy; c.in_ch = p->c_out; c.srcH = p->h_out; c.srcW = p->w_out; c.out_ch = 4 * p->c_in;
    c.tm = TapMap{2, 2, 0, 2, 0, 2, 1, p->c_in};
    c.PH = (p->h_in + 1) / 2; c.PW = (p->w_in + 1) / 2;
    c.h_mul = 1; c.tap_h_mul = -1; c.h_off = 0;
    c.w_mul = 1; c.rep_mul = -1; c.w_off = 0;
    c.out_H = p->h_in; c.out_W = p->w_in; c.oh_mul = 2; c.oh_off = 0; c.ow_mul = 2; c.ow_off = 0;
    c.fuse = p->c_in;
    return plan_problem(c, p->batch, p->precision).ok;
}

int umma_dy_replicas(const cpc_conv_params* p) {
    if (p->stride_h == 1 && p->stride_w == 1) return 1;
    if (!umma_conv_eligible(p, 1)) return 1;
    ConvProblem f;
    if (fused_dgrad_problem(nullptr, p, f)) return 2;
    const DgradShare d = dgrad_share(p);
    return (d.common && d.n_classes > 1 && d.max_tw == 2 && d.w_off == 0) ? 2 : 1;
}
static int dy_packed_wp(const cpc_conv_params* p, int nrep) { return (p->w_out + (nrep == 2 ? 1 : 0) + 7) & ~7; }

size_t umma_conv_workspace(const cpc_conv_params* p, int which) {
    if (!umma_conv_eligible(p, which)) return 0;
    size_t need = 0;
    if (which == 0) {
        UmmaPlan u = plan_problem(fwd_problem(nullptr, p), p->batch, p->precision);
        need = u.act_bytes + u.w_bytes;
    } else {
        const DgradShare d = dgrad_share(p);
        need = d.max_single;
        if (d.common && d.act_bytes + d.max_w_bytes > need) need = d.act_bytes + d.max_w_bytes;
        ConvProblem f;
        if (fused_dgrad_problem(nullptr, p, f)) {
            UmmaPlan u = plan_problem(f, p->batch, p->precision);
            if (u.act_bytes + u.w_bytes > need) need = u.act_bytes + u.w_bytes;
        }
    }
    return need + 2048;
}

int umma_conv_launch(const float* in, const float* w, const float* bias, float* out, const cpc_conv_params* p, int which,
                     const void* pre, void* workspace, size_t workspace_bytes, cudaStream_t s) {
    const __nv_bfloat16* prep = reinterpret_cast<const __nv_bfloat16*>(pre);
    if (which == 0) {
        ConvProblem c = fwd_problem(in, p);
        if (prep) { c.pre = prep; c.pre_Wp = (p->w_out + 7) & ~7; c.pre_nrep = p->kw; }
        return run_problem(c, w, bias, out, p, p->relu, workspace, workspace_bytes, s);
    }
    const int pre_rep = prep ? umma_dy_replicas(p) : 1;
    {
        ConvProblem f;
        if (fused_dgrad_problem(in, p, f)) {
            if (prep && pre_rep == 2) { f.pre = prep; f.pre_Wp = dy_packed_wp(p, 2); f.pre_nrep = 2; }
            return run_problem(f, w, nullptr, out, p, 0, workspace, workspace_bytes, s);
        }
    }
    bool need_zero = false;
    for (int rh = 0; rh < p->stride_h; ++rh)
        for (int rw = 0; rw < p->stride_w; ++rw) {
            ConvProblem c; bool taps;
            if (dgrad_problem(in, p, rh, rw, c, taps) && !taps) need_zero = true;
        }
    if (need_zero &&
        cudaMemsetAsync(out, 0, sizeof(float) * (size_t)p->batch * p->c_in * p->h_in * p->w_in, s) != cudaSuccess)
        return CPC_ERR_CUDA;
    const DgradShare d = dgrad_share(p);
    const int pre_Wp = (p->w_out + 7) & ~7;
    const bool use_pre = prep && pre_rep == 1 && d.common && d.max_tw == 1 && d.w_off == 0 && d.max_pw <= pre_Wp;
    const bool use_pre2 = prep && pre_rep == 2 && d.common && d.max_tw <= 2 && d.w_off == 0;
    const __nv_bfloat16* shared = nullptr;
    int shared_Wp = 0, shared_nrep = 0;
    uint8_t* ws = reinterpret_cast<uint8_t*>(workspace);
    size_t ws_bytes = workspace_bytes;
    if (use_pre) {
        shared = prep; shared_Wp = pre_Wp; shared_nrep = 1;
    } else if (use_pre2) {
        shared = prep; shared_Wp = dy_packed_wp(p, 2); shared_nrep = 2;
    } else if (d.common && d.n_classes > 1) {
        if (!workspace || workspace_bytes < d.act_bytes + d.max_w_bytes + 2048) return CPC_ERR_WORKSPACE;
        uint8_t* base = reinterpret_cast<uint8_t*>((reinterpret_cast<uintptr_t>(workspace) + 1023) & ~(uintptr_t)1023);
        shared_Wp = (d.max_pw + 7) & ~7;
        shared_nrep = d.max_tw;
        const int planes = p->precision == 1 ? 1 : 2;
        if (pack_split_launch(in, reinterpret_cast<__nv_bfloat16*>(base), (long)p->batch * p->c_out * p->h_out, p->w_out,
                              shared_Wp, planes, shared_nrep, 1, -1, d.w_off, s) != CPC_OK)
            return CPC_ERR_CUDA;
        count_launch();
        shared = reinterpret_cast<const __nv_bfloat16*>(base);
        ws = base + d.act_bytes;
        ws_bytes = workspace_bytes - (size_t)(ws - reinterpret_cast<uint8_t*>(workspace));
    }
    for (int rh = 0; rh < p->stride_h; ++rh)
        for (int rw = 0; rw < p->stride_w; ++rw) {
            ConvProblem c; bool taps;
            if (!dgrad_problem(in, p, rh, rw, c, taps) || !taps) continue;
            if (shared) { c.pre = shared; c.pre_Wp = shared_Wp; c.pre_nrep = shared_nrep; }
            const int st = run_problem(c, w, nullptr, out, p, 0, ws, ws_bytes, s);
            if (st != CPC_OK) return st;
        }
    return CPC_OK;
}


struct UmmaWgrad {
    int OH, AW, B;
    int n_chunks_total, chunks_per_split, n_splits;
    int n_xtiles, n_ntiles, n_tile;
    int CB, TH, cin, cout, kh, kw;
    int c_tiles, h_tiles;
    int pt, sh, planes, stages;
    float* dw;
};

__global__ void __launch_bounds__(UM_THREADS, 1) umma_wgrad_kernel(const __grid_constant__ CUtensorMap tmap_x,
                                                                  const __grid_constant__ CUtensorMap tmap_dy,
                                                                  const UmmaWgrad p) {
    extern __shared__ __align__(1024) uint8_t smem_raw[];
    uint8_t* smem = reinterpret_cast<uint8_t*>((reinterpret_cast<uintptr_t>(smem_raw) + 1023) & ~(uintptr_t)1023);
    constexpr int A_BYTES = 128 * 128;
    const int b_bytes = p.n_tile * 128;
    const int stage_bytes = p.planes * (A_BYTES + b_bytes);
    UmmaBarriers* bars = reinterpret_cast<UmmaBarriers*>(smem + (size_t)p.stages * stage_bytes);
    const int warp = threadIdx.x >> 5, lane = threadIdx.x & 31;

    int t = blockIdx.x;
    const int ntile = t % p.n_ntiles; t /= p.n_ntiles;
    const int xtile = t % p.n_xtiles;
    const int j = t / p.n_xtiles;
    const int ctile = xtile / p.h_tiles, htile = xtile - ctile * p.h_tiles;
    const int c0 = ctile * p.CB, i0 = htile * p.TH;
    const int q_begin = blockIdx.y * p.chunks_per_split;
    const int q_end = min(p.n_chunks_total, q_begin + p.chunks_per_split);
    const int nq = q_end - q_begin;

    if (warp == 0 && lane == 0) {
        prefetch_tmap(&tmap_x);
        prefetch_tmap(&tmap_dy);
        for (int s = 0; s < p.stages; ++s) { mbar_init(&bars->full[s], 1); mbar_init(&bars->empty[s], 1); }
        mbar_init(&bars->acc_full[0], 1);
        fence_barrier_init();
    }
    if (warp == 2) { tmem_alloc(&bars->tmem_base, 256); tmem_relinquish(); }
    tc_fence_before();
    __syncthreads();
    tc_fence_after();
    const uint32_t tmem_base = bars->tmem_base;

    if (warp == 0) {
        int stage = 0; uint32_t phase = 0;
        int wa, b, oh;
        {
            const int row = q_begin / p.AW;
            wa = q_begin - row * p.AW;
            b = row / p.OH; oh = row - b * p.OH;
        }
        for (int q = q_begin; q < q_end; ++q) {
            const int w0 = wa * ATOM;
            if (lane == 0) {
                mbar_wait(&bars->empty[stage], phase ^ 1);
                mbar_expect_tx(&bars->full[stage], (uint32_t)stage_bytes);
            }
            __syncwarp();
            uint8_t* st = smem + (size_t)stage * stage_bytes;
            if (lane < 2 * p.planes) {
                const int pl = lane >> 1;
                if ((lane & 1) == 0)
                    tma_load_5d(st + pl * A_BYTES, &tmap_x, &bars->full[stage], w0, oh * p.sh + i0 - p.pt, c0, b, pl * p.kw + j);
                else
                    tma_load_5d(st + p.planes * A_BYTES + pl * b_bytes, &tmap_dy, &bars->full[stage], w0, oh, ntile * p.n_tile,
                                b, pl);
            }
            if (++wa == p.AW) { wa = 0; if (++oh == p.OH) { oh = 0; ++b; } }
            if (++stage == p.stages) { stage = 0; phase ^= 1; }
        }
    } else if (warp == 1) {
        if (lane == 0) {
            const uint32_t idesc = make_idesc_bf16(128, p.n_tile, 0, 0);
            int stage = 0; uint32_t phase = 0;
            for (int q = 0; q < nq; ++q) {
                mbar_wait(&bars->full[stage], phase);
                tc_fence_after();
                const uint32_t st = smem_u32(smem + (size_t)stage * stage_bytes);
                const uint32_t b0 = st + p.planes * A_BYTES;
                const int ncombo = p.planes == 2 ? 3 : 1;
                for (int cb = 0; cb < ncombo; ++cb) {
                    const uint64_t a_d = make_smem_desc(st + (cb == 2 ? A_BYTES : 0), 16, 1024);
                    const uint64_t b_d = make_smem_desc(b0 + (cb == 1 ? b_bytes : 0), 16, 1024);
#pragma unroll
                    for (int k = 0; k < 4; ++k)
                        mma_bf16(tmem_base, a_d + (uint64_t)(k * 2), b_d + (uint64_t)(k * 2), idesc, (q | cb | k) != 0);
                }
                tc_commit(&bars->empty[stage]);
                if (++stage == p.stages) { stage = 0; phase ^= 1; }
            }
            tc_commit(&bars->acc_full[0]);
        }
    } else if (warp >= 4) {
        const int ew = warp & 3;
        const int m = ew * 32 + lane;
        const int ci = c0 + m / p.TH, i = i0 + m % p.TH;
        const bool valid = nq > 0 && ci < p.cin && i < p.kh;
        mbar_wait(&bars->acc_full[0], 0);
        tc_fence_after();
        const uint32_t taddr = tmem_base + ((uint32_t)(ew * 32) << 16);
        for (int n0 = 0; n0 < p.n_tile; n0 += 32) {
            uint32_t v[32];
            tmem_ld32(taddr + n0, v);
            tmem_ld_wait();
            if (valid) {
#pragma unroll
                for (int c = 0; c < 32; ++c) {
                    const int co = ntile * p.n_tile + n0 + c;
                    atomicAdd(p.dw + (((size_t)co * p.cin + ci) * p.kh + i) * p.kw + j, __uint_as_float(v[c]));
                }
            }
        }
    }
    tc_fence_before();
    __syncthreads();
    if (warp == 2) { tc_fence_after(); tmem_dealloc(tmem_base, 256); }
}

struct WgradPlan {
    bool ok;
    int CB, TH, c_tiles, h_tiles, n_tile, n_ntiles, planes, stages, Wp_x, Wp_dy, AW;
    size_t x_bytes, dy_bytes, smem_bytes;
};

static WgradPlan make_wgrad_plan(const cpc_conv_params* p) {
    WgradPlan u{};
    u.ok = false;
    if (p->stride_h > 8 || p->stride_w > 8) return u;
    const int ci = p->c_in, co = p->c_out;
    if (!(ci == 16 || ci == 32 || ci == 64 || ci % 128 == 0)) return u;
    if (co % 32 != 0 || !(co <= 256 || co % 256 == 0)) return u;
    u.CB = ci < 128 ? ci : 128;
    u.TH = 128 / u.CB;
    u.c_tiles = ci / u.CB;
    u.h_tiles = (p->kh + u.TH - 1) / u.TH;
    u.n_tile = co <= 256 ? co : 256;
    u.n_ntiles = co / u.n_tile;
    u.planes = p->precision == 1 ? 1 : 2;
    u.Wp_x = (p->w_out + 7) & ~7;
    u.Wp_dy = (p->w_out + 7) & ~7;
    u.AW = (p->w_out + ATOM - 1) / ATOM;
    if ((long)p->batch * p->h_out * u.AW > (1l << 30)) return u;
    const int stage_bytes = u.planes * (128 * 128 + u.n_tile * 128);
    u.stages = (SMEM_LIMIT - 2048) / stage_bytes;
    if (u.stages > 8) u.stages = 8;
    if (u.stages < 2) return u;
    u.smem_bytes = (size_t)u.stages * stage_bytes + sizeof(UmmaBarriers) + 1024;
    u.x_bytes = align_up((size_t)u.planes * p->kw * p->batch * ci * p->h_in * u.Wp_x * 2, 1024);
    u.dy_bytes = align_up((size_t)u.planes * p->batch * co * p->h_out * u.Wp_dy * 2, 1024);
    u.ok = true;
    return u;
}

size_t umma_wgrad_workspace(const cpc_conv_params* p) {
    WgradPlan u = make_wgrad_plan(p);
    return u.ok ? u.x_bytes + u.dy_bytes + 1024 : 0;
}
bool umma_wgrad_eligible(const cpc_conv_params* p) { return make_wgrad_plan(p).ok; }

int umma_wgrad_launch(const float* x, const float* dy, float* dw, const cpc_conv_params* p, const void* pre_x,
                      const void* pre_dy, void* workspace, size_t workspace_bytes, cudaStream_t s) {
    WgradPlan u = make_wgrad_plan(p);
    if (!u.ok) return CPC_ERR_UNSUPPORTED;
    if (!workspace || workspace_bytes < u.x_bytes + u.dy_bytes + 1024) return CPC_ERR_WORKSPACE;
    uint8_t* ws = reinterpret_cast<uint8_t*>((reinterpret_cast<uintptr_t>(workspace) + 1023) & ~(uintptr_t)1023);
    const __nv_bfloat16* xp = pre_x ? reinterpret_cast<const __nv_bfloat16*>(pre_x) : reinterpret_cast<__nv_bfloat16*>(ws);
    const __nv_bfloat16* dyp =
        pre_dy ? reinterpret_cast<const __nv_bfloat16*>(pre_dy) : reinterpret_cast<__nv_bfloat16*>(ws + u.x_bytes);
    const int B = p->batch;
    {
        const long rows_x = (long)B * p->c_in * p->h_in;
        if (!pre_x && pack_split_launch(x, reinterpret_cast<__nv_bfloat16*>(ws), rows_x, p->w_in, u.Wp_x, u.planes, p->kw,
                                        p->stride_w, 1, -p->pad_left, s) != CPC_OK)
            return CPC_ERR_CUDA;
        const long rows_dy = (long)B * p->c_out * p->h_out;
        if (!pre_dy && pack_split_launch(dy, reinterpret_cast<__nv_bfloat16*>(ws + u.x_bytes), rows_dy, p->w_out, u.Wp_dy,
                                         u.planes, 1, 1, 0, 0, s) != CPC_OK)
            return CPC_ERR_CUDA;
    }
    CUtensorMap tx, tdy;
    {
        const uint64_t rb = (uint64_t)u.Wp_x * 2;
        const uint64_t dims[5] = {(uint64_t)u.Wp_x, (uint64_t)p->h_in, (uint64_t)p->c_in, (uint64_t)B,
                                  (uint64_t)u.planes * p->kw};
        const uint64_t strides[4] = {rb, rb * p->h_in, rb * p->h_in * p->c_in, rb * p->h_in * p->c_in * B};
        const uint32_t box[5] = {ATOM, (uint32_t)u.TH, (uint32_t)u.CB, 1, 1};
        if (!make_tmap_bf16(&tx, xp, 5, dims, strides, box)) return CPC_ERR_CUDA;
        const int dy_rep = pre_dy ? umma_dy_replicas(p) : 1;
        const uint64_t rd = (uint64_t)(pre_dy ? dy_packed_wp(p, dy_rep) : u.Wp_dy) * 2;
        const uint64_t ddims[5] = {(uint64_t)p->w_out, (uint64_t)p->h_out, (uint64_t)p->c_out, (uint64_t)B,
                                   (uint64_t)u.planes};
        const uint64_t dstr[4] = {rd, rd * p->h_out, rd * p->h_out * p->c_out, rd * p->h_out * p->c_out * B * dy_rep};
        const uint32_t dbox[5] = {ATOM, 1, (uint32_t)u.n_tile, 1, 1};
        if (!make_tmap_bf16(&tdy, dyp, 5, ddims, dstr, dbox)) return CPC_ERR_CUDA;
    }
    UmmaWgrad k{};
    k.OH = p->h_out; k.AW = u.AW; k.B = B;
    k.n_chunks_total = B * p->h_out * u.AW;
    k.n_xtiles = u.c_tiles * u.h_tiles; k.n_ntiles = u.n_ntiles; k.n_tile = u.n_tile;
    k.CB = u.CB; k.TH = u.TH; k.cin = p->c_in; k.cout = p->c_out; k.kh = p->kh; k.kw = p->kw;
    k.c_tiles = u.c_tiles; k.h_tiles = u.h_tiles;
    k.pt = p->pad_top; k.sh = p->stride_h; k.planes = u.planes; k.stages = u.stages;
    k.dw = dw;
    const int tiles = k.n_xtiles * k.n_ntiles * p->kw;
    int splits = 148 / tiles;
    const int max_splits = (k.n_chunks_total + 15) / 16;
    if (splits > max_splits) splits = max_splits;
    if (splits < 1) splits = 1;
    k.chunks_per_split = (k.n_chunks_total + splits - 1) / splits;
    k.n_splits = (k.n_chunks_total + k.chunks_per_split - 1) / k.chunks_per_split;
    if (cudaMemsetAsync(dw, 0, sizeof(float) * (size_t)p->c_out * p->c_in * p->kh * p->kw, s) != cudaSuccess)
        return CPC_ERR_CUDA;
    if (cudaFuncSetAttribute(umma_wgrad_kernel, cudaFuncAttributeMaxDynamicSharedMemorySize, SMEM_LIMIT) != cudaSuccess)
        return CPC_ERR_CUDA;
    umma_wgrad_kernel<<<dim3(tiles, k.n_splits), UM_THREADS, u.smem_bytes, s>>>(tx, tdy, k);
    CPC_LAUNCH_CHECK();
    count_launch(3);
    return CPC_OK;
}

}
```

Before: 31000.

## Fuse fp32-to-bf16 operand packing into UMMA conv and wgrad producer warps

```diff
diff --git a/constrastive-predictive-coding-audio_b200/cpc_b200/ops.py b/constrastive-predictive-coding-audio_b200/cpc_b200/ops.py
--- a/constrastive-predictive-coding-audio_b200/cpc_b200/ops.py
+++ b/constrastive-predictive-coding-audio_b200/cpc_b200/ops.py
@@ -175,8 +175,16 @@
     return p
 
 
+def _packed_bytes(lib, p, operand):
+    nbytes = lib.cpc_conv_packed_bytes(ctypes.byref(p), operand)
+    if nbytes == 0 or _switch("CPC_PACK_CONV_OPERANDS"):
+        return nbytes
+    readers = (0, 2) if operand == 0 else (1, 2)
+    return nbytes if any(lib.cpc_conv_kernel_family(ctypes.byref(p), w) in (2, 3) for w in readers) else 0
+
+
 def _pack_operand(lib, t, p, operand):
-    nbytes = lib.cpc_conv_packed_bytes(ctypes.byref(p), operand)
+    nbytes = _packed_bytes(lib, p, operand)
     if nbytes == 0:
         return None
     packed = torch.empty(int(nbytes), dtype=torch.uint8, device=t.device)
@@ -285,7 +293,7 @@
     with torch.cuda.device(dy.device):
         packed_dy = None
         if need_dw:
-            nbytes = lib.cpc_conv_packed_bytes(ctypes.byref(p), 1)
+            nbytes = _packed_bytes(lib, p, 1)
             if nbytes and ctx.has_bias:
                 packed_dy = torch.empty(int(nbytes), dtype=torch.uint8, device=dy.device)
                 db = torch.empty(w_shape[0], dtype=torch.float32, device=dy.device)
diff --git a/constrastive-predictive-coding-audio_b200/csrc/conv.cu b/constrastive-predictive-coding-audio_b200/csrc/conv.cu
--- a/constrastive-predictive-coding-audio_b200/csrc/conv.cu
+++ b/constrastive-predictive-coding-audio_b200/csrc/conv.cu
@@ -15,10 +15,9 @@
                           int nrep, cudaStream_t s);
 int umma_dy_replicas(const cpc_conv_params* p);
 
-size_t umma_wgrad_workspace(const cpc_conv_params* p);
 bool umma_wgrad_eligible(const cpc_conv_params* p);
-int umma_wgrad_launch(const float* x, const float* dy, float* dw, const cpc_conv_params* p, const void* pre_x,
-                      const void* pre_dy, void* workspace, size_t workspace_bytes, cudaStream_t s);
+int umma_wgrad_launch(const float* x, const float* dy, float* dw, float* dbias, const cpc_conv_params* p, const void* pre_x,
+                      const void* pre_dy, cudaStream_t s);
 
 size_t tall_conv_workspace(const cpc_conv_params* p, int which);
 bool tall_conv_eligible(const cpc_conv_params* p, int which);
@@ -266,7 +265,6 @@
     if (which >= 0 && which <= 2 && tall_path(p, which))
         return tall_path(p, which) == 1 ? tall_conv_workspace(p, which) : tall128_workspace(p, which);
     if ((which == 0 || which == 1) && tensor_core_path(p, which)) return umma_conv_workspace(p, which);
-    if (which == 2 && tensor_core_path(p, 2)) return umma_wgrad_workspace(p);
     return 0;
 }
 
@@ -438,7 +436,11 @@
         if (fam == 1) st = smallk_launch(2, x, nullptr, nullptr, dy, dw, p, s);
         else if (fam == 2) st = tall_wgrad_launch(x, dy, dw, p, packed_x, packed_dy, workspace, workspace_bytes, s);
         else if (fam == 3) st = tall128_wgrad_launch(x, dy, dw, p, packed_x, packed_dy, workspace, workspace_bytes, s);
-        else st = umma_wgrad_launch(x, dy, dw, p, packed_x, packed_dy, workspace, workspace_bytes, s);
+        else {
+            st = umma_wgrad_launch(x, dy, dw, packed_dy ? nullptr : dbias, p, packed_x, packed_dy, s);
+            if (st != CPC_OK) return st;
+            return dbias && packed_dy ? launch_dbias(dy, dbias, g, s) : CPC_OK;
+        }
         if (st != CPC_OK) return st;
         return dbias ? launch_dbias(dy, dbias, g, s) : CPC_OK;
     }
diff --git a/constrastive-predictive-coding-audio_b200/csrc/conv_umma.cu b/constrastive-predictive-coding-audio_b200/csrc/conv_umma.cu
--- a/constrastive-predictive-coding-audio_b200/csrc/conv_umma.cu
+++ b/constrastive-predictive-coding-audio_b200/csrc/conv_umma.cu
@@ -26,7 +26,82 @@
     int relu, stages;
     const float* bias;
     float* y;
+    const float* src;
+    int B, in_ch, srcW, w_mul, rep_mul, w_off;
 };
+
+constexpr int CVT_WARPS = 8;
+constexpr int CVT_ROWS = 16;
+constexpr int UM_THREADS_DIRECT = UM_THREADS + 32 * CVT_WARPS;
+
+template <class Row>
+__device__ __forceinline__ void cvt_load(float (&v)[2 * CVT_ROWS], Row row, int col0, int col1, bool ok0, bool ok1,
+                                         bool vec) {
+    if (vec && ok0 && ok1) {
+#pragma unroll
+        for (int r = 0; r < CVT_ROWS; ++r) {
+            const float* q;
+            const bool live = row(r, q);
+            const float2 t = live ? __ldg(reinterpret_cast<const float2*>(q + col0)) : make_float2(0.f, 0.f);
+            v[2 * r] = t.x; v[2 * r + 1] = t.y;
+        }
+    } else {
+#pragma unroll
+        for (int r = 0; r < CVT_ROWS; ++r) {
+            const float* q;
+            const bool live = row(r, q);
+            v[2 * r] = live && ok0 ? __ldg(q + col0) : 0.f;
+            v[2 * r + 1] = live && ok1 ? __ldg(q + col1) : 0.f;
+        }
+    }
+}
+
+__device__ __forceinline__ void sts32(uint32_t addr, __nv_bfloat162 v) {
+    asm volatile("st.shared.b32 [%0], %1;" ::"r"(addr), "r"(*reinterpret_cast<uint32_t*>(&v)) : "memory");
+}
+
+__device__ __forceinline__ void cvt_store(const float (&v)[2 * CVT_ROWS], uint8_t* dst, int plane_bytes, int planes, int lane) {
+    const uint32_t base = smem_u32(dst) + ((uint32_t)(lane & 3) << 2);
+#pragma unroll
+    for (int r = 0; r < CVT_ROWS; ++r) {
+        const __nv_bfloat162 hi = __floats2bfloat162_rn(v[2 * r], v[2 * r + 1]);
+        const uint32_t a = base + (uint32_t)r * 128 + ((uint32_t)((lane >> 2) ^ (r & 7)) << 4);
+        sts32(a, hi);
+        if (planes == 2) {
+            const float2 h = __bfloat1622float2(hi);
+            sts32(a + plane_bytes, __floats2bfloat162_rn(v[2 * r] - h.x, v[2 * r + 1] - h.y));
+        }
+    }
+}
+
+__device__ __forceinline__ float row_sums_to_lanes(const float (&v)[2 * CVT_ROWS], int lane) {
+    float t[CVT_ROWS];
+#pragma unroll
+    for (int r = 0; r < CVT_ROWS; ++r) t[r] = v[2 * r] + v[2 * r + 1];
+#pragma unroll
+    for (int w = CVT_ROWS / 2; w >= 1; w >>= 1) {
+        const bool upper = (lane & (2 * w)) != 0;
+#pragma unroll
+        for (int k = 0; k < w; ++k) {
+            const float keep = upper ? t[k + w] : t[k], send = upper ? t[k] : t[k + w];
+            t[k] = keep + __shfl_xor_sync(0xffffffffu, send, 2 * w);
+        }
+    }
+    return t[0] + __shfl_xor_sync(0xffffffffu, t[0], 1);
+}
+
+template <class Load, class Store>
+__device__ __forceinline__ void cvt_pipeline(Load&& load, Store&& store) {
+    float va[2 * CVT_ROWS], vb[2 * CVT_ROWS];
+    bool ha = load(va);
+    while (ha) {
+        const bool hb = load(vb);
+        store(va);
+        if (!hb) break;
+        ha = load(va);
+        store(vb);
+    }
+}
 
 __global__ void __launch_bounds__(256) pack_split_kernel(const float* __restrict__ x, __nv_bfloat16* __restrict__ out,
                                                         long rows, int W, int Wp, int planes, int nrep, int w_mul,
@@ -260,9 +335,9 @@
     uint32_t tmem_base;
 };
 
-__global__ void __launch_bounds__(UM_THREADS, 1) umma_conv_kernel(const __grid_constant__ CUtensorMap tmap_a,
-                                                                 const __grid_constant__ CUtensorMap tmap_b,
-                                                                 const UmmaConv p) {
+__global__ void __launch_bounds__(UM_THREADS_DIRECT, 1) umma_conv_kernel(const __grid_constant__ CUtensorMap tmap_a,
+                                                                        const __grid_constant__ CUtensorMap tmap_b,
+                                                                        const UmmaConv p) {
     extern __shared__ __align__(1024) uint8_t smem_raw[];
     uint8_t* smem = reinterpret_cast<uint8_t*>((reinterpret_cast<uintptr_t>(smem_raw) + 1023) & ~(uintptr_t)1023);
     const int b_plane_bytes = p.n_tile * 128;
@@ -276,10 +351,11 @@
     const int n_mtiles = (p.n_atoms + 1) >> 1;
     const int n_tiles = n_mtiles * p.n_ntiles;
 
+    const bool direct = p.src != nullptr;
     if (warp == 0 && lane == 0) {
-        prefetch_tmap(&tmap_a);
+        if (!direct) prefetch_tmap(&tmap_a);
         prefetch_tmap(&tmap_b);
-        for (int s = 0; s < p.stages; ++s) { mbar_init(&bars->full[s], 1); mbar_init(&bars->empty[s], 1); }
+        for (int s = 0; s < p.stages; ++s) { mbar_init(&bars->full[s], direct ? 1 + CVT_WARPS : 1); mbar_init(&bars->empty[s], 1); }
         for (int b = 0; b < 2; ++b) { mbar_init(&bars->acc_full[b], 1); mbar_init(&bars->acc_empty[b], 4); }
         mbar_init(&bars->wfull, 1);
         fence_barrier_init();
@@ -300,8 +376,9 @@
             }
         }
         const int taps_per_load = p.cin_eff == KCHUNK ? 1 : p.tpc;
-        const int n_a_loads = p.planes * 2 * taps_per_load;
+        const int n_a_loads = direct ? 0 : p.planes * 2 * taps_per_load;
         const int n_loads = n_a_loads + (p.w_resident ? 0 : p.planes);
+        const uint32_t tx_bytes = (uint32_t)(direct ? stage_bytes - p.planes * A_PLANE_BYTES : stage_bytes);
         const bool is_a = lane < n_a_loads, is_b = !is_a && lane < n_loads;
         const int my_t = is_a ? lane % taps_per_load : 0;
         const int my_a = is_a ? (lane / taps_per_load) & 1 : 0;
@@ -331,7 +408,7 @@
             for (int q = q_begin; q < q_end; ++q) {
                 if (lane == 0) {
                     mbar_wait(&bars->empty[stage], phase ^ 1);
-                    mbar_expect_tx(&bars->full[stage], (uint32_t)stage_bytes);
+                    mbar_expect_tx(&bars->full[stage], tx_bytes);
                 }
                 __syncwarp();
                 uint8_t* dst = stages_base + (size_t)stage * stage_bytes + my_off;
@@ -398,6 +475,65 @@
                 if (++buf == 2) { buf = 0; acc_phase ^= 1; }
             }
         }
+    } else if (warp >= 8) {
+        const int cw = warp - 8;
+        const int a = cw >> 2, krow0 = (cw & 3) * CVT_ROWS;
+        const int t_in = p.cin_eff == KCHUNK ? 0 : krow0 / p.cin_eff;
+        const int c_in = p.cin_eff == KCHUNK ? krow0 : krow0 - t_in * p.cin_eff;
+        const size_t plane = (size_t)p.srcH * p.srcW;
+        const bool vec_ok = p.w_mul == 1 && (p.srcW & 1) == 0 && (reinterpret_cast<uintptr_t>(p.src) & 7) == 0;
+        int lt = (int)blockIdx.x - (int)gridDim.x, left = 0;
+        int ti = 0, tj = 0, cc = 0, hrow = 0, cbase = 0;
+        bool b_ok = false;
+        const float* tile_src = p.src;
+        auto load = [&](float (&v)[2 * CVT_ROWS]) -> bool {
+            if (left == 0) {
+                if ((lt += gridDim.x) >= n_tiles) return false;
+                const int mtile = lt / p.n_ntiles;
+                int aoh[2];
+                for (int e = 0; e < 2; ++e) {
+                    const int row = (mtile * 2 + e) / p.AW;
+                    aoh[e] = (row - (row / p.PH) * p.PH) * p.h_mul + p.h_off;
+                }
+                int q_begin, q_end;
+                umma_live_chunks(p, aoh[0], aoh[1], q_begin, q_end);
+                left = q_end - q_begin;
+                const int atom = mtile * 2 + a, row = atom / p.AW, b = row / p.PH;
+                hrow = aoh[a];
+                b_ok = b < p.B;
+                tile_src = p.src + (size_t)b * p.in_ch * plane;
+                cbase = p.w_mul * ((atom - row * p.AW) * ATOM + 2 * lane) + p.w_off;
+                const int tap = p.cin_eff == KCHUNK ? q_begin / p.cin_chunks : q_begin * p.tpc + t_in;
+                cc = p.cin_eff == KCHUNK ? q_begin - tap * p.cin_chunks : 0;
+                ti = tap / p.tw; tj = tap - ti * p.tw;
+            }
+            --left;
+            const int c0 = cc * KCHUNK + c_in;
+            const int h = hrow + ti * p.tap_h_mul;
+            const bool live = b_ok && ti < p.th && h >= 0 && h < p.srcH;
+            const float* base = tile_src + ((size_t)c0 * p.srcH + h) * p.srcW;
+            const int col0 = cbase + p.rep_mul * tj, col1 = col0 + p.w_mul;
+            cvt_load(v, [&](int r, const float*& q) { q = base + r * plane; return live; }, col0, col1,
+                     col0 >= 0 && col0 < p.srcW, col1 >= 0 && col1 < p.srcW, vec_ok && !(col0 & 1));
+            if (p.cin_eff == KCHUNK) {
+                if (++cc == p.cin_chunks) { cc = 0; if (++tj == p.tw) { tj = 0; ++ti; } }
+            } else {
+                tj += p.tpc;
+                while (tj >= p.tw) { tj -= p.tw; ++ti; }
+            }
+            return true;
+        };
+        int stage = 0; uint32_t phase = 0;
+        auto store = [&](const float (&v)[2 * CVT_ROWS]) {
+            mbar_wait(&bars->empty[stage], phase ^ 1);
+            cvt_store(v, stages_base + (size_t)stage * stage_bytes + a * (KCHUNK * 128) + krow0 * 128, A_PLANE_BYTES,
+                      p.planes, lane);
+            fence_proxy_async();
+            __syncwarp();
+            if (lane == 0) mbar_arrive(&bars->full[stage]);
+            if (++stage == p.stages) { stage = 0; phase ^= 1; }
+        };
+        cvt_pipeline(load, store);
     } else if (warp >= 4) {
         const int ew = warp & 3;
         const int r = ew * 32 + lane;
@@ -483,7 +619,7 @@
 struct UmmaPlan {
     bool ok;
     int Wp, cin_eff, cin_chunks, tpc, n_chunks, n_tile, n_ntiles, planes, stages, w_resident;
-    size_t act_bytes, w_bytes, smem_bytes;
+    size_t w_bytes, smem_bytes;
 };
 
 static UmmaPlan plan_problem(const ConvProblem& c, int batch, int precision) {
@@ -512,7 +648,6 @@
     if (u.stages > 8) u.stages = 8;
     if (u.stages < 2) return u;
     u.smem_bytes = (size_t)(u.w_resident ? w_all : 0) + (size_t)u.stages * stage_bytes + sizeof(UmmaBarriers) + 1024;
-    u.act_bytes = c.pre ? 0 : align_up((size_t)u.planes * c.tm.tw * batch * ci * c.srcH * u.Wp * 2, 1024);
     u.w_bytes = align_up((size_t)u.planes * u.n_chunks * co * KCHUNK * 2, 1024);
     u.ok = true;
     return u;
@@ -523,16 +658,11 @@
     const int B = p->batch;
     UmmaPlan u = plan_problem(c, B, p->precision);
     if (!u.ok) return CPC_ERR_UNSUPPORTED;
-    if (!workspace || workspace_bytes < u.act_bytes + u.w_bytes + 1024) return CPC_ERR_WORKSPACE;
+    if (!workspace || workspace_bytes < u.w_bytes + 1024) return CPC_ERR_WORKSPACE;
     uint8_t* ws = reinterpret_cast<uint8_t*>((reinterpret_cast<uintptr_t>(workspace) + 1023) & ~(uintptr_t)1023);
-    const __nv_bfloat16* act = c.pre ? c.pre : reinterpret_cast<__nv_bfloat16*>(ws);
-    __nv_bfloat16* wp = reinterpret_cast<__nv_bfloat16*>(ws + u.act_bytes);
-    const long rows = (long)B * c.in_ch * c.srcH;
+    __nv_bfloat16* wp = reinterpret_cast<__nv_bfloat16*>(ws);
     const int nrep = c.pre ? c.pre_nrep : c.tm.tw;
     {
-        if (!c.pre && pack_split_launch(c.src, reinterpret_cast<__nv_bfloat16*>(ws), rows, c.srcW, u.Wp, u.planes, c.tm.tw,
-                                        c.w_mul, c.rep_mul, c.w_off, s) != CPC_OK)
-            return CPC_ERR_CUDA;
         const long wtotal = (long)u.n_chunks * c.out_ch * KCHUNK;
         int wblocks = (int)((wtotal + 255) / 256);
         if (wblocks > 148 * 8) wblocks = 148 * 8;
@@ -540,14 +670,14 @@
                                                     u.cin_chunks, u.tpc, u.n_chunks, u.planes, c.tm);
         CPC_LAUNCH_CHECK();
     }
-    CUtensorMap ta, tb;
+    CUtensorMap ta{}, tb;
     {
         const uint64_t dims[5] = {(uint64_t)u.Wp, (uint64_t)c.srcH, (uint64_t)c.in_ch, (uint64_t)B,
                                   (uint64_t)u.planes * nrep};
         const uint64_t row_b = (uint64_t)u.Wp * 2;
         const uint64_t strides[4] = {row_b, row_b * c.srcH, row_b * c.srcH * c.in_ch, row_b * c.srcH * c.in_ch * B};
         const uint32_t box[5] = {ATOM, 1, (uint32_t)u.cin_eff, 1, 1};
-        if (!make_tmap_bf16(&ta, act, 5, dims, strides, box)) return CPC_ERR_CUDA;
+        if (c.pre && !make_tmap_bf16(&ta, c.pre, 5, dims, strides, box)) return CPC_ERR_CUDA;
         const uint64_t wd[4] = {KCHUNK, (uint64_t)c.out_ch, (uint64_t)u.n_chunks, (uint64_t)u.planes};
         const uint64_t wsr[3] = {KCHUNK * 2, (uint64_t)KCHUNK * 2 * c.out_ch, (uint64_t)KCHUNK * 2 * c.out_ch * u.n_chunks};
         const uint32_t wbox[4] = {KCHUNK, (uint32_t)u.n_tile, 1, 1};
@@ -564,13 +694,17 @@
     k.out_H = c.out_H; k.out_W = c.out_W; k.oh_mul = c.oh_mul; k.oh_off = c.oh_off; k.ow_mul = c.ow_mul; k.ow_off = c.ow_off;
     k.fuse = c.fuse;
     k.planes = u.planes; k.nrep = nrep; k.w_resident = u.w_resident; k.relu = relu; k.stages = u.stages; k.bias = bias; k.y = out; k.srcH = c.srcH;
+    if (!c.pre) {
+        k.src = c.src; k.B = B; k.in_ch = c.in_ch; k.srcW = c.srcW;
+        k.w_mul = c.w_mul; k.rep_mul = c.rep_mul; k.w_off = c.w_off;
+    }
     if (cudaFuncSetAttribute(umma_conv_kernel, cudaFuncAttributeMaxDynamicSharedMemorySize, SMEM_LIMIT) != cudaSuccess)
         return CPC_ERR_CUDA;
     const int n_tiles = ((k.n_atoms + 1) / 2) * k.n_ntiles;
     const int grid = n_tiles < 148 ? n_tiles : 148;
-    umma_conv_kernel<<<grid, UM_THREADS, u.smem_bytes, s>>>(ta, tb, k);
+    umma_conv_kernel<<<grid, c.pre ? UM_THREADS : UM_THREADS_DIRECT, u.smem_bytes, s>>>(ta, tb, k);
     CPC_LAUNCH_CHECK();
-    count_launch(c.pre ? 2 : 3);
+    count_launch(2);
     return CPC_OK;
 }
 
@@ -627,9 +761,7 @@
 struct DgradShare {
     bool common;
     int n_classes, max_tw, max_pw, w_off;
-    size_t act_bytes;
     size_t max_w_bytes;
-    size_t max_single;
 };
 
 static DgradShare dgrad_share(const cpc_conv_params* p) {
@@ -647,11 +779,7 @@
             if (c.tm.tw > d.max_tw) d.max_tw = c.tm.tw;
             if (c.PW > d.max_pw) d.max_pw = c.PW;
             if (u.w_bytes > d.max_w_bytes) d.max_w_bytes = u.w_bytes;
-            if (u.act_bytes + u.w_bytes > d.max_single) d.max_single = u.act_bytes + u.w_bytes;
-        }
-    const int planes = p->precision == 1 ? 1 : 2;
-    const int Wp = (d.max_pw + 7) & ~7;
-    d.act_bytes = align_up((size_t)planes * d.max_tw * p->batch * p->c_out * p->h_out * Wp * 2, 1024);
+        }
     return d;
 }
 
@@ -684,16 +812,13 @@
     if (!umma_conv_eligible(p, which)) return 0;
     size_t need = 0;
     if (which == 0) {
-        UmmaPlan u = plan_problem(fwd_problem(nullptr, p), p->batch, p->precision);
-        need = u.act_bytes + u.w_bytes;
+        need = plan_problem(fwd_problem(nullptr, p), p->batch, p->precision).w_bytes;
     } else {
-        const DgradShare d = dgrad_share(p);
-        need = d.max_single;
-        if (d.common && d.act_bytes + d.max_w_bytes > need) need = d.act_bytes + d.max_w_bytes;
+        need = dgrad_share(p).max_w_bytes;
         ConvProblem f;
         if (fused_dgrad_problem(nullptr, p, f)) {
-            UmmaPlan u = plan_problem(f, p->batch, p->precision);
-            if (u.act_bytes + u.w_bytes > need) need = u.act_bytes + u.w_bytes;
+            const size_t wb = plan_problem(f, p->batch, p->precision).w_bytes;
+            if (wb > need) need = wb;
         }
     }
     return need + 2048;
@@ -730,32 +855,17 @@
     const bool use_pre2 = prep && pre_rep == 2 && d.common && d.max_tw <= 2 && d.w_off == 0;
     const __nv_bfloat16* shared = nullptr;
     int shared_Wp = 0, shared_nrep = 0;
-    uint8_t* ws = reinterpret_cast<uint8_t*>(workspace);
-    size_t ws_bytes = workspace_bytes;
     if (use_pre) {
         shared = prep; shared_Wp = pre_Wp; shared_nrep = 1;
     } else if (use_pre2) {
         shared = prep; shared_Wp = dy_packed_wp(p, 2); shared_nrep = 2;
-    } else if (d.common && d.n_classes > 1) {
-        if (!workspace || workspace_bytes < d.act_bytes + d.max_w_bytes + 2048) return CPC_ERR_WORKSPACE;
-        uint8_t* base = reinterpret_cast<uint8_t*>((reinterpret_cast<uintptr_t>(workspace) + 1023) & ~(uintptr_t)1023);
-        shared_Wp = (d.max_pw + 7) & ~7;
-        shared_nrep = d.max_tw;
-        const int planes = p->precision == 1 ? 1 : 2;
-        if (pack_split_launch(in, reinterpret_cast<__nv_bfloat16*>(base), (long)p->batch * p->c_out * p->h_out, p->w_out,
-                              shared_Wp, planes, shared_nrep, 1, -1, d.w_off, s) != CPC_OK)
-            return CPC_ERR_CUDA;
-        count_launch();
-        shared = reinterpret_cast<const __nv_bfloat16*>(base);
-        ws = base + d.act_bytes;
-        ws_bytes = workspace_bytes - (size_t)(ws - reinterpret_cast<uint8_t*>(workspace));
     }
     for (int rh = 0; rh < p->stride_h; ++rh)
         for (int rw = 0; rw < p->stride_w; ++rw) {
             ConvProblem c; bool taps;
             if (!dgrad_problem(in, p, rh, rw, c, taps) || !taps) continue;
             if (shared) { c.pre = shared; c.pre_Wp = shared_Wp; c.pre_nrep = shared_nrep; }
-            const int st = run_problem(c, w, nullptr, out, p, 0, ws, ws_bytes, s);
+            const int st = run_problem(c, w, nullptr, out, p, 0, workspace, workspace_bytes, s);
             if (st != CPC_OK) return st;
         }
     return CPC_OK;
@@ -770,11 +880,15 @@
     int c_tiles, h_tiles;
     int pt, sh, planes, stages;
     float* dw;
+    const float* x;
+    const float* dy;
+    float* dbias;
+    int H, W, OW, sw, pl, cvt_warps;
 };
 
-__global__ void __launch_bounds__(UM_THREADS, 1) umma_wgrad_kernel(const __grid_constant__ CUtensorMap tmap_x,
-                                                                  const __grid_constant__ CUtensorMap tmap_dy,
-                                                                  const UmmaWgrad p) {
+__global__ void __launch_bounds__(UM_THREADS_DIRECT, 1) umma_wgrad_kernel(const __grid_constant__ CUtensorMap tmap_x,
+                                                                         const __grid_constant__ CUtensorMap tmap_dy,
+                                                                         const UmmaWgrad p) {
     extern __shared__ __align__(1024) uint8_t smem_raw[];
     uint8_t* smem = reinterpret_cast<uint8_t*>((reinterpret_cast<uintptr_t>(smem_raw) + 1023) & ~(uintptr_t)1023);
     constexpr int A_BYTES = 128 * 128;
@@ -794,9 +908,9 @@
     const int nq = q_end - q_begin;
 
     if (warp == 0 && lane == 0) {
-        prefetch_tmap(&tmap_x);
-        prefetch_tmap(&tmap_dy);
-        for (int s = 0; s < p.stages; ++s) { mbar_init(&bars->full[s], 1); mbar_init(&bars->empty[s], 1); }
+        if (!p.x) prefetch_tmap(&tmap_x);
+        if (!p.dy) prefetch_tmap(&tmap_dy);
+        for (int s = 0; s < p.stages; ++s) { mbar_init(&bars->full[s], 1 + p.cvt_warps); mbar_init(&bars->empty[s], 1); }
         mbar_init(&bars->acc_full[0], 1);
         fence_barrier_init();
     }
@@ -807,6 +921,8 @@
     const uint32_t tmem_base = bars->tmem_base;
 
     if (warp == 0) {
+        const uint32_t tx_bytes = (uint32_t)((p.x ? 0 : p.planes * A_BYTES) + (p.dy ? 0 : p.planes * b_bytes));
+        const bool my_load = lane < 2 * p.planes && ((lane & 1) ? !p.dy : !p.x);
         int stage = 0; uint32_t phase = 0;
         int wa, b, oh;
         {
@@ -818,11 +934,11 @@
             const int w0 = wa * ATOM;
             if (lane == 0) {
                 mbar_wait(&bars->empty[stage], phase ^ 1);
-                mbar_expect_tx(&bars->full[stage], (uint32_t)stage_bytes);
+                mbar_expect_tx(&bars->full[stage], tx_bytes);
             }
             __syncwarp();
             uint8_t* st = smem + (size_t)stage * stage_bytes;
-            if (lane < 2 * p.planes) {
+            if (my_load) {
                 const int pl = lane >> 1;
                 if ((lane & 1) == 0)
                     tma_load_5d(st + pl * A_BYTES, &tmap_x, &bars->full[stage], w0, oh * p.sh + i0 - p.pt, c0, b, pl * p.kw + j);
@@ -855,6 +971,79 @@
             }
             tc_commit(&bars->acc_full[0]);
         }
+    } else if (warp >= 8) {
+        const int cw = warp - 8, nw = p.cvt_warps;
+        const int gx = p.x ? 128 / CVT_ROWS : 0;
+        const int G = gx + (p.dy ? p.n_tile / CVT_ROWS : 0);
+        const int my_groups = (G - cw + nw - 1) / nw;
+        const int x_slots = gx ? 1 : 0;
+        const int th_shift = __ffs(p.TH) - 1;
+        const bool vec_x = p.sw == 1 && (p.W & 1) == 0 && (reinterpret_cast<uintptr_t>(p.x) & 7) == 0;
+        const bool vec_dy = (p.OW & 1) == 0 && (reinterpret_cast<uintptr_t>(p.dy) & 7) == 0;
+        const bool sum_bias = p.dbias && p.dy && j == 0 && xtile == 0;
+        float bacc0 = 0.f, bacc1 = 0.f;
+        int lq = q_begin, lk = -1, wa, oh, bi;
+        {
+            const int row = q_begin / p.AW;
+            wa = q_begin - row * p.AW; bi = row / p.OH; oh = row - bi * p.OH;
+        }
+        const size_t x_plane = (size_t)p.H * p.W, dy_plane = (size_t)p.OH * p.OW;
+        auto load = [&](float (&v)[2 * CVT_ROWS]) -> bool {
+            if (++lk == my_groups) {
+                lk = 0; ++lq;
+                if (++wa == p.AW) { wa = 0; if (++oh == p.OH) { oh = 0; ++bi; } }
+            }
+            if (lq >= q_end) return false;
+            const int pw = wa * ATOM + 2 * lane;
+            const int g = cw + lk * nw;
+            if (g < gx) {
+                const int m0 = g * CVT_ROWS;
+                const int col0 = p.sw * pw + j - p.pl, col1 = col0 + p.sw;
+                const float* xb = p.x + (size_t)bi * p.cin * x_plane;
+                const int h0 = oh * p.sh - p.pt;
+                cvt_load(v, [&](int r, const float*& q) {
+                    const int m = m0 + r, c = c0 + (m >> th_shift), i = i0 + (m & (p.TH - 1));
+                    const int h = h0 + i;
+                    q = xb + (size_t)c * x_plane + (size_t)h * p.W;
+                    return i < p.kh && h >= 0 && h < p.H;
+                }, col0, col1, pw < p.OW && col0 >= 0 && col0 < p.W, pw + 1 < p.OW && col1 >= 0 && col1 < p.W,
+                         vec_x && !(col0 & 1));
+            } else {
+                const float* db = p.dy + ((size_t)bi * p.cout + ntile * p.n_tile + (g - gx) * CVT_ROWS) * dy_plane +
+                                  (size_t)oh * p.OW;
+                cvt_load(v, [&](int r, const float*& q) { q = db + r * dy_plane; return true; }, pw, pw + 1, pw < p.OW,
+                         pw + 1 < p.OW, vec_dy);
+            }
+            return true;
+        };
+        int sk = -1, stage = 0; uint32_t phase = 0;
+        auto store = [&](const float (&v)[2 * CVT_ROWS]) {
+            if (++sk == my_groups) { sk = 0; if (++stage == p.stages) { stage = 0; phase ^= 1; } }
+            const int g = cw + sk * nw;
+            if (sk == 0) mbar_wait(&bars->empty[stage], phase ^ 1);
+            uint8_t* st = smem + (size_t)stage * stage_bytes;
+            if (g < gx) {
+                cvt_store(v, st + g * (CVT_ROWS * 128), A_BYTES, p.planes, lane);
+            } else {
+                cvt_store(v, st + p.planes * A_BYTES + (g - gx) * (CVT_ROWS * 128), b_bytes, p.planes, lane);
+                if (sum_bias) {
+                    const float t = row_sums_to_lanes(v, lane);
+                    if (sk == x_slots) bacc0 += t; else bacc1 += t;
+                }
+            }
+            if (sk == my_groups - 1) {
+                fence_proxy_async();
+                __syncwarp();
+                if (lane == 0) mbar_arrive(&bars->full[stage]);
+            }
+        };
+        cvt_pipeline(load, store);
+        if (sum_bias && !(lane & 1)) {
+            for (int ds = 0; ds < 2 && x_slots + ds < my_groups; ++ds) {
+                const int co0 = ntile * p.n_tile + (cw + (x_slots + ds) * nw - gx) * CVT_ROWS;
+                atomicAdd(p.dbias + co0 + (lane >> 1), ds == 0 ? bacc0 : bacc1);
+            }
+        }
     } else if (warp >= 4) {
         const int ew = warp & 3;
         const int m = ew * 32 + lane;
@@ -883,8 +1072,8 @@
 
 struct WgradPlan {
     bool ok;
-    int CB, TH, c_tiles, h_tiles, n_tile, n_ntiles, planes, stages, Wp_x, Wp_dy, AW;
-    size_t x_bytes, dy_bytes, smem_bytes;
+    int CB, TH, c_tiles, h_tiles, n_tile, n_ntiles, planes, stages, Wp, AW;
+    size_t smem_bytes;
 };
 
 static WgradPlan make_wgrad_plan(const cpc_conv_params* p) {
@@ -901,8 +1090,7 @@
     u.n_tile = co <= 256 ? co : 256;
     u.n_ntiles = co / u.n_tile;
     u.planes = p->precision == 1 ? 1 : 2;
-    u.Wp_x = (p->w_out + 7) & ~7;
-    u.Wp_dy = (p->w_out + 7) & ~7;
+    u.Wp = (p->w_out + 7) & ~7;
     u.AW = (p->w_out + ATOM - 1) / ATOM;
     if ((long)p->batch * p->h_out * u.AW > (1l << 30)) return u;
     const int stage_bytes = u.planes * (128 * 128 + u.n_tile * 128);
@@ -910,53 +1098,35 @@
     if (u.stages > 8) u.stages = 8;
     if (u.stages < 2) return u;
     u.smem_bytes = (size_t)u.stages * stage_bytes + sizeof(UmmaBarriers) + 1024;
-    u.x_bytes = align_up((size_t)u.planes * p->kw * p->batch * ci * p->h_in * u.Wp_x * 2, 1024);
-    u.dy_bytes = align_up((size_t)u.planes * p->batch * co * p->h_out * u.Wp_dy * 2, 1024);
     u.ok = true;
     return u;
 }
 
-size_t umma_wgrad_workspace(const cpc_conv_params* p) {
-    WgradPlan u = make_wgrad_plan(p);
-    return u.ok ? u.x_bytes + u.dy_bytes + 1024 : 0;
-}
 bool umma_wgrad_eligible(const cpc_conv_params* p) { return make_wgrad_plan(p).ok; }
 
-int umma_wgrad_launch(const float* x, const float* dy, float* dw, const cpc_conv_params* p, const void* pre_x,
-                      const void* pre_dy, void* workspace, size_t workspace_bytes, cudaStream_t s) {
+int umma_wgrad_launch(const float* x, const float* dy, float* dw, float* dbias, const cpc_conv_params* p, const void* pre_x,
+                      const void* pre_dy, cudaStream_t s) {
     WgradPlan u = make_wgrad_plan(p);
     if (!u.ok) return CPC_ERR_UNSUPPORTED;
-    if (!workspace || workspace_bytes < u.x_bytes + u.dy_bytes + 1024) return CPC_ERR_WORKSPACE;
-    uint8_t* ws = reinterpret_cast<uint8_t*>((reinterpret_cast<uintptr_t>(workspace) + 1023) & ~(uintptr_t)1023);
-    const __nv_bfloat16* xp = pre_x ? reinterpret_cast<const __nv_bfloat16*>(pre_x) : reinterpret_cast<__nv_bfloat16*>(ws);
-    const __nv_bfloat16* dyp =
-        pre_dy ? reinterpret_cast<const __nv_bfloat16*>(pre_dy) : reinterpret_cast<__nv_bfloat16*>(ws + u.x_bytes);
+    if (dbias && pre_dy) return CPC_ERR_UNSUPPORTED;
     const int B = p->batch;
-    {
-        const long rows_x = (long)B * p->c_in * p->h_in;
-        if (!pre_x && pack_split_launch(x, reinterpret_cast<__nv_bfloat16*>(ws), rows_x, p->w_in, u.Wp_x, u.planes, p->kw,
-                                        p->stride_w, 1, -p->pad_left, s) != CPC_OK)
-            return CPC_ERR_CUDA;
-        const long rows_dy = (long)B * p->c_out * p->h_out;
-        if (!pre_dy && pack_split_launch(dy, reinterpret_cast<__nv_bfloat16*>(ws + u.x_bytes), rows_dy, p->w_out, u.Wp_dy,
-                                         u.planes, 1, 1, 0, 0, s) != CPC_OK)
-            return CPC_ERR_CUDA;
-    }
-    CUtensorMap tx, tdy;
-    {
-        const uint64_t rb = (uint64_t)u.Wp_x * 2;
-        const uint64_t dims[5] = {(uint64_t)u.Wp_x, (uint64_t)p->h_in, (uint64_t)p->c_in, (uint64_t)B,
+    CUtensorMap tx{}, tdy{};
+    if (pre_x) {
+        const uint64_t rb = (uint64_t)u.Wp * 2;
+        const uint64_t dims[5] = {(uint64_t)u.Wp, (uint64_t)p->h_in, (uint64_t)p->c_in, (uint64_t)B,
                                   (uint64_t)u.planes * p->kw};
         const uint64_t strides[4] = {rb, rb * p->h_in, rb * p->h_in * p->c_in, rb * p->h_in * p->c_in * B};
         const uint32_t box[5] = {ATOM, (uint32_t)u.TH, (uint32_t)u.CB, 1, 1};
-        if (!make_tmap_bf16(&tx, xp, 5, dims, strides, box)) return CPC_ERR_CUDA;
-        const int dy_rep = pre_dy ? umma_dy_replicas(p) : 1;
-        const uint64_t rd = (uint64_t)(pre_dy ? dy_packed_wp(p, dy_rep) : u.Wp_dy) * 2;
+        if (!make_tmap_bf16(&tx, pre_x, 5, dims, strides, box)) return CPC_ERR_CUDA;
+    }
+    if (pre_dy) {
+        const int dy_rep = umma_dy_replicas(p);
+        const uint64_t rd = (uint64_t)dy_packed_wp(p, dy_rep) * 2;
         const uint64_t ddims[5] = {(uint64_t)p->w_out, (uint64_t)p->h_out, (uint64_t)p->c_out, (uint64_t)B,
                                    (uint64_t)u.planes};
         const uint64_t dstr[4] = {rd, rd * p->h_out, rd * p->h_out * p->c_out, rd * p->h_out * p->c_out * B * dy_rep};
         const uint32_t dbox[5] = {ATOM, 1, (uint32_t)u.n_tile, 1, 1};
-        if (!make_tmap_bf16(&tdy, dyp, 5, ddims, dstr, dbox)) return CPC_ERR_CUDA;
+        if (!make_tmap_bf16(&tdy, pre_dy, 5, ddims, dstr, dbox)) return CPC_ERR_CUDA;
     }
     UmmaWgrad k{};
     k.OH = p->h_out; k.AW = u.AW; k.B = B;
@@ -966,6 +1136,12 @@
     k.c_tiles = u.c_tiles; k.h_tiles = u.h_tiles;
     k.pt = p->pad_top; k.sh = p->stride_h; k.planes = u.planes; k.stages = u.stages;
     k.dw = dw;
+    k.x = pre_x ? nullptr : x;
+    k.dy = pre_dy ? nullptr : dy;
+    k.dbias = dbias;
+    k.H = p->h_in; k.W = p->w_in; k.OW = p->w_out; k.sw = p->stride_w; k.pl = p->pad_left;
+    const int groups = (k.x ? 128 / CVT_ROWS : 0) + (k.dy ? u.n_tile / CVT_ROWS : 0);
+    k.cvt_warps = groups < CVT_WARPS ? groups : CVT_WARPS;
     const int tiles = k.n_xtiles * k.n_ntiles * p->kw;
     int splits = 148 / tiles;
     const int max_splits = (k.n_chunks_total + 15) / 16;
@@ -975,11 +1151,12 @@
     k.n_splits = (k.n_chunks_total + k.chunks_per_split - 1) / k.chunks_per_split;
     if (cudaMemsetAsync(dw, 0, sizeof(float) * (size_t)p->c_out * p->c_in * p->kh * p->kw, s) != cudaSuccess)
         return CPC_ERR_CUDA;
+    if (dbias && cudaMemsetAsync(dbias, 0, sizeof(float) * (size_t)p->c_out, s) != cudaSuccess) return CPC_ERR_CUDA;
     if (cudaFuncSetAttribute(umma_wgrad_kernel, cudaFuncAttributeMaxDynamicSharedMemorySize, SMEM_LIMIT) != cudaSuccess)
         return CPC_ERR_CUDA;
-    umma_wgrad_kernel<<<dim3(tiles, k.n_splits), UM_THREADS, u.smem_bytes, s>>>(tx, tdy, k);
+    umma_wgrad_kernel<<<dim3(tiles, k.n_splits), UM_THREADS + 32 * k.cvt_warps, u.smem_bytes, s>>>(tx, tdy, k);
     CPC_LAUNCH_CHECK();
-    count_launch(3);
+    count_launch(1);
     return CPC_OK;
 }
 
```

After: 25200 (median of 6 runs). -18.7%, worse.
